# ATTron/astroz

Measured on AMD Instinct MI355X. Metric: propagations/sec, 13,478 sats x 1,440 times, at 1/2/4/8 MI355X, higher is better.
Workload: dtype f64

## Files before the change

astroz_amd/_native.py:

```python
import ctypes as C
import os

import numpy as np

_HERE = os.path.dirname(os.path.abspath(__file__))
LIB_PATH = os.environ.get("ASTROZ_AMD_LIB") or os.path.join(_HERE, "libastroz_hip.so")

WGS84, WGS72 = 0, 1
OUT_TEME, OUT_ECEF, OUT_GEODETIC, OUT_TOPOCENTRIC = 0, 1, 2, 3
SAT_MAJOR, TIME_MAJOR = 0, 1
OUTPUT_MODES = {"teme": OUT_TEME, "ecef": OUT_ECEF, "geodetic": OUT_GEODETIC, "topocentric": OUT_TOPOCENTRIC}
PASS_DTYPE = np.dtype([("t_rise_min", "<f8"), ("t_culm_min", "<f8"), ("t_set_min", "<f8"), ("max_elevation_rad", "<f8"),
                       ("rise_azimuth_rad", "<f8"), ("set_azimuth_rad", "<f8"), ("flags", "<u4"), ("grid_rise", "<u4"),
                       ("grid_culm", "<u4"), ("grid_set", "<u4")])
PASS_UP_AT_START, PASS_UP_AT_END, PASS_CUT_BY_ERROR = 1, 2, 4
ECLIPSE_DTYPE = np.dtype([("t_entry_min", "<f8"), ("t_exit_min", "<f8"), ("flags", "<u4"), ("grid_entry", "<u4"),
                          ("grid_exit", "<u4"), ("reserved", "<u4")])
ECLIPSE_IN_AT_START, ECLIPSE_IN_AT_END, ECLIPSE_CUT_BY_ERROR = 1, 2, 4
SHADOW_UMBRA, SHADOW_PENUMBRA = 0, 1
SHADOW_KINDS = {"umbra": SHADOW_UMBRA, "penumbra": SHADOW_PENUMBRA}
ACCESS_DTYPE = np.dtype([("t_start_min", "<f8"), ("t_end_min", "<f8"), ("min_range_km", "<f8"), ("flags", "<u4"),
                         ("grid_start", "<u4"), ("grid_end", "<u4"), ("grid_min_range", "<u4")])
ACCESS_OPEN_AT_START, ACCESS_OPEN_AT_END, ACCESS_CUT_BY_ERROR = 1, 2, 4
CONJUNCTION_DTYPE = np.dtype([("t_tca_min", "<f8"), ("miss_km", "<f8"), ("rel_speed_km_s", "<f8"), ("target", "<u4"),
                              ("sat", "<u4"), ("grid_index", "<u4"), ("reserved", "<u4")])

COVERAGE_DTYPE = np.dtype([("mean_in_view", "<f8"), ("max_gap_min", "<f8"), ("n_covered", "<u4"), ("min_in_view", "<u4"),
                           ("max_in_view", "<u4"), ("n_gaps", "<u4"), ("grid_gap_start", "<u4"), ("grid_gap_end", "<u4"),
                           ("flags", "<u4"), ("reserved", "<u4")])
COVERAGE_GAP_AT_START, COVERAGE_GAP_AT_END = 1, 2

AZ_ERR_HIP = -200
PATH_ROWS_FAST, PATH_TILES_FAST, PATH_ROWS_GENERIC, PATH_LANE_SAT, PATH_DEEP_ROWS, PATH_QUASI_UNIFORM, PATH_COLS_FAST, PATH_HOST_STEP = 1, 2, 4, 8, 16, 32, 64, 128

EXPORTS = [
    "astroz_version", "astroz_init", "astroz_deinit", "tle_parse", "tle_free",
    "tle_get_satellite_number", "tle_get_epoch", "tle_get_inclination", "tle_get_eccentricity",
    "tle_get_mean_motion", "sgp4_init", "sgp4_free", "sgp4_propagate", "sgp4_propagate_batch",
    "azh_device_count", "azh_last_error", "azh_parse_tle_lines", "azh_constellation_from_tle_text",
    "azh_constellation_from_tle_lines", "azh_constellation_from_elements", "azh_constellation_subset", "azh_constellation_free",
    "azh_num_satellites", "azh_num_sgp4", "azh_num_sdp4", "azh_get_epochs", "azh_get_status",
    "azh_get_field", "azh_propagate_host", "azh_propagate_device", "azh_propagate_device_cached", "azh_propagate_device_window",
    "azh_propagate_jd_host", "azh_synchronize", "azh_propagate_one_host", "azh_set_time_tile", "azh_set_timing", "azh_set_fast_path", "azh_set_tile_kernel", "azh_set_graphs", "azh_set_f32_arithmetic", "azh_set_f32_mode",
    "azh_last_kernel_ms", "azh_last_path", "azh_last_one_stats", "azh_set_host_copy_threads", "azh_set_host_points", "azh_get_host_points", "azh_selftest_coords", "azh_selftest_host_step", "azh_host_alloc", "azh_host_free", "azh_host_pool_stats", "azh_host_pool_trim", "azh_propagate_device_f32", "azh_propagate_device_cached_f32",
    "azh_screen_target_host", "azh_screen_target_device", "azh_coarse_screen_device", "azh_coarse_screen_host",
    "azh_screen_all_host", "azh_constellation_from_omm_json", "azh_propagate_one_device", "azh_selftest_math",
    "azh_parse_tle_text", "azh_parse_omm_json", "azh_set_parse_threads", "coords_julian_to_gmst",
    "azh_group_create_from_tle_text", "azh_group_create_from_omm_json", "azh_group_free", "azh_group_num_satellites",
    "azh_group_num_devices", "azh_group_padded_rows", "azh_group_get_epochs", "azh_group_propagate_host",
    "azh_group_propagate_allgather", "azh_group_screen_target_host", "azh_group_screen_target_device", "azh_group_shard_size",
    "azh_group_shard_rows", "azh_group_synchronize", "azh_screen_track_device", "coords_eci_to_ecef", "coords_ecef_to_geodetic",
    "orbital_hohmann", "orbital_velocity", "orbital_period", "orbital_escape_velocity",
    "azh_coords_topocentric", "azh_set_observer", "azh_find_passes_host", "azh_find_passes_device",
    "azh_find_passes_stations_host", "azh_find_passes_stations_device",
    "azh_coverage_host", "azh_coverage_device",
    "azh_sun_position_teme", "azh_selftest_sun", "azh_shadow_state", "azh_find_eclipses_host", "azh_find_eclipses_device",
    "azh_line_of_sight", "azh_find_access_host", "azh_find_access_device", "azh_find_access_track_device",
    "azh_closest_approach", "azh_find_conjunctions_host", "azh_find_conjunctions_device",
]


def _stations(stations, min_elevation_deg):
    st = np.ascontiguousarray(stations, dtype=np.float64).reshape(-1, 3)
    mk = np.ascontiguousarray(np.broadcast_to(np.asarray(min_elevation_deg, dtype=np.float64), (len(st),)))
    return st, mk


def _targets(targets):
    a = np.atleast_1d(np.asarray(targets))
    if a.ndim != 1 or a.size == 0 or a.dtype == np.bool_ or not np.issubdtype(a.dtype, np.integer) or (a < 0).any():
        raise ValueError("targets must be a satellite index or a non-empty sequence of them")
    return np.ascontiguousarray(a, dtype=np.uintp)


def _min_satellites(k):
    if isinstance(k, bool) or not isinstance(k, (int, np.integer)) or not 1 <= int(k) <= 0xFFFFFFFF:
        raise ValueError("min_satellites must be an integer >= 1")
    return int(k)


class NativeError(RuntimeError):
    def __init__(self, code, what):
        self.code = code
        super().__init__("%s failed with code %d%s" % (what, code, _detail(code)))


_lib = None


def _detail(code):
    if _lib is not None and code == AZ_ERR_HIP:
        msg = _lib.azh_last_error().decode(errors="replace")
        return " (%s)" % msg if msg else " (HIP runtime error: is an MI355X visible?)"
    return ""


def _share_hip_runtime_with_torch():
    if os.environ.get("ASTROZ_AMD_SYSTEM_HIP"):
        return
    import importlib.util
    try:
        spec = importlib.util.find_spec("torch")
    except (ImportError, ValueError):
        spec = None
    if spec is None or not spec.origin:
        return
    cand = os.path.join(os.path.dirname(spec.origin), "lib", "libamdhip64.so")
    if os.path.exists(cand):
        C.CDLL(cand, mode=C.RTLD_GLOBAL)


def lib():
    global _lib
    if _lib is not None:
        return _lib
    if not os.path.exists(LIB_PATH):
        raise ImportError(
            "astroz_amd: %s not found -- build it with `python -c 'import __graft_entry__ as g; "
            "g.build()'` (hipcc --offload-arch=gfx950). There is no CPU fallback." % LIB_PATH)
    _share_hip_runtime_with_torch()
    L = C.CDLL(LIB_PATH)
    vp, sz, dbl, i32, u32 = C.c_void_p, C.c_size_t, C.c_double, C.c_int32, C.c_uint32
    L.astroz_version.restype = u32
    L.tle_parse.argtypes = [C.c_char_p, C.POINTER(vp)]
    L.tle_parse.restype = i32
    L.tle_free.argtypes = [vp]
    L.tle_get_satellite_number.argtypes = [vp]
# ... 41 lines not shown
    L.azh_group_screen_target_device.restype = i32
    L.azh_group_shard_size.argtypes = [vp, i32]
    L.azh_group_shard_size.restype = sz
    L.azh_group_shard_rows.argtypes = [vp, i32, vp]
    L.azh_group_shard_rows.restype = i32
    L.azh_group_synchronize.argtypes = [vp]
    L.azh_group_synchronize.restype = i32
    L.azh_constellation_from_omm_json.argtypes = [C.c_char_p, sz, i32, i32, C.POINTER(vp)]
    L.azh_constellation_from_omm_json.restype = i32
    L.azh_propagate_one_device.argtypes = [vp, sz, vp, sz, vp, vp, vp, vp]
    L.azh_propagate_one_device.restype = i32
    L.azh_selftest_math.argtypes = [vp, sz, vp, i32]
    L.azh_selftest_math.restype = i32
    L.coords_julian_to_gmst.argtypes = [dbl]
    L.coords_julian_to_gmst.restype = dbl
    L.coords_eci_to_ecef.argtypes = [vp, dbl, vp]
    L.coords_eci_to_ecef.restype = None
    L.coords_ecef_to_geodetic.argtypes = [vp, vp]
    L.coords_ecef_to_geodetic.restype = None
    L.azh_constellation_from_tle_lines.argtypes = [vp, vp, sz, i32, i32, C.POINTER(vp)]
    L.azh_constellation_from_tle_lines.restype = i32
    L.azh_constellation_from_elements.argtypes = [sz] + [vp] * 8 + [i32, i32, C.POINTER(vp)]
    L.azh_constellation_from_elements.restype = i32
    L.azh_constellation_subset.argtypes = [vp, vp, sz, i32, C.POINTER(vp)]
    L.azh_constellation_subset.restype = i32
    L.azh_constellation_free.argtypes = [vp]
    for f in ("azh_num_satellites", "azh_num_sgp4", "azh_num_sdp4"):
        getattr(L, f).argtypes = [vp]
        getattr(L, f).restype = sz
    L.azh_get_epochs.argtypes = [vp, vp]
    L.azh_get_epochs.restype = i32
    L.azh_get_status.argtypes = [vp, vp, vp, vp]
    L.azh_get_status.restype = i32
    L.azh_get_field.argtypes = [vp, C.c_char_p, vp]
    L.azh_get_field.restype = i32
    L.azh_propagate_host.argtypes = [vp, vp, sz, vp, vp, vp, i32, dbl, vp, i32, sz, vp]
    L.azh_propagate_host.restype = i32
    L.azh_propagate_device.argtypes = [vp, vp, sz, vp, vp, vp, i32, dbl, vp, i32, sz, vp, vp]
    L.azh_propagate_device.restype = i32
    L.azh_propagate_device_cached.argtypes = [vp, vp, vp, i32, sz, vp, vp]
    L.azh_propagate_device_cached.restype = i32
    L.azh_propagate_device_window.argtypes = [vp, sz, sz, vp, vp, i32, sz, vp, vp]
    L.azh_propagate_device_window.restype = i32
    L.azh_propagate_jd_host.argtypes = [vp, vp, vp, sz, vp, vp, i32, i32, vp]
    L.azh_propagate_jd_host.restype = i32
    L.azh_synchronize.argtypes = [vp]
    L.azh_synchronize.restype = i32
    L.azh_propagate_one_host.argtypes = [vp, sz, vp, sz, vp, vp, vp]
    L.azh_propagate_one_host.restype = i32
    L.azh_set_time_tile.argtypes = [vp, u32, u32]
    L.azh_set_time_tile.restype = i32
    L.azh_set_timing.argtypes = [vp, i32]
    L.azh_set_timing.restype = i32
    L.azh_set_fast_path.argtypes = [vp, i32]
    L.azh_set_fast_path.restype = i32
    L.azh_set_tile_kernel.argtypes = [vp, i32]
    L.azh_set_tile_kernel.restype = i32
    L.azh_set_graphs.argtypes = [vp, i32]
    L.azh_set_graphs.restype = i32
    L.azh_set_f32_arithmetic.argtypes = [vp, i32]
    L.azh_set_f32_arithmetic.restype = i32
    L.azh_set_f32_mode.argtypes = [vp, i32]
    L.azh_set_f32_mode.restype = i32
    L.azh_last_kernel_ms.argtypes = [vp]
    L.azh_last_kernel_ms.restype = dbl
    L.azh_set_host_copy_threads.argtypes = [i32]
    L.azh_set_host_copy_threads.restype = None
    L.azh_set_host_points.argtypes = [sz]
    L.azh_set_host_points.restype = None
    L.azh_get_host_points.argtypes = []
    L.azh_get_host_points.restype = sz
    L.azh_host_alloc.argtypes = [C.c_size_t, C.POINTER(C.c_void_p)]
    L.azh_host_alloc.restype = i32
    L.azh_host_free.argtypes = [C.c_void_p]
    L.azh_host_free.restype = None
    L.azh_host_pool_stats.argtypes = [C.POINTER(C.c_size_t), C.POINTER(C.c_size_t)]
    L.azh_host_pool_stats.restype = None
    L.azh_host_pool_trim.argtypes = []
    L.azh_host_pool_trim.restype = None
    L.azh_last_path.argtypes = [vp]
    L.azh_last_path.restype = u32
    L.azh_last_one_stats.argtypes = [vp, vp, vp]
    L.azh_last_one_stats.restype = C.c_int32
    L.azh_propagate_device_f32.argtypes = L.azh_propagate_device.argtypes
    L.azh_propagate_device_f32.restype = i32
    L.azh_propagate_device_cached_f32.argtypes = L.azh_propagate_device_cached.argtypes
    L.azh_propagate_device_cached_f32.restype = i32
    L.azh_screen_target_host.argtypes = [vp, vp, sz, vp, sz, dbl, dbl, vp, vp]
    L.azh_screen_target_host.restype = i32
    L.azh_screen_target_device.argtypes = [vp, vp, sz, vp, sz, dbl, dbl, vp, vp, vp]
    L.azh_screen_target_device.restype = i32
    L.azh_screen_track_device.argtypes = [vp, vp, sz, vp, vp, sz, dbl, vp, vp, vp]
    L.azh_screen_track_device.restype = i32
    L.azh_coarse_screen_device.argtypes = [vp, sz, sz, i32, sz, dbl, vp, vp, vp, sz, C.POINTER(sz), vp]
    L.azh_coarse_screen_device.restype = i32
    L.azh_coarse_screen_host.argtypes = [vp, sz, sz, i32, sz, dbl, vp, vp, vp, sz, C.POINTER(sz), i32]
    L.azh_coarse_screen_host.restype = i32
    L.azh_screen_all_host.argtypes = [vp, vp, sz, vp, dbl, vp, vp, sz, C.POINTER(sz)]
    L.azh_screen_all_host.restype = i32
    L.azh_coords_topocentric.argtypes = [vp, vp, dbl, vp, vp, vp]
    L.azh_coords_topocentric.restype = None
    L.azh_set_observer.argtypes = [vp, dbl, dbl, dbl]
    L.azh_set_observer.restype = i32
    L.azh_find_passes_host.argtypes = [vp, vp, sz, vp, dbl, dbl, vp, sz, vp]
    L.azh_find_passes_host.restype = i32
    L.azh_find_passes_device.argtypes = [vp, vp, sz, vp, dbl, dbl, vp, sz, vp, vp]
    L.azh_find_passes_device.restype = i32
    L.azh_find_passes_stations_host.argtypes = [vp, vp, sz, vp, dbl, vp, vp, sz, vp, sz, vp]
    L.azh_find_passes_stations_host.restype = i32
    L.azh_find_passes_stations_device.argtypes = [vp, vp, sz, vp, dbl, vp, vp, sz, vp, sz, vp, vp]
    L.azh_find_passes_stations_device.restype = i32
    L.azh_coverage_host.argtypes = [vp, vp, sz, vp, dbl, vp, vp, sz, u32, vp, vp]
    L.azh_coverage_host.restype = i32
    L.azh_coverage_device.argtypes = [vp, vp, sz, vp, dbl, vp, vp, sz, u32, vp, vp, vp]
    L.azh_coverage_device.restype = i32
    L.azh_sun_position_teme.argtypes = [dbl, vp]
    L.azh_sun_position_teme.restype = None
    L.azh_selftest_sun.argtypes = [vp, sz, vp, i32]
    L.azh_selftest_sun.restype = i32
    L.azh_shadow_state.argtypes = [vp, vp, vp, vp]
    L.azh_shadow_state.restype = i32
    L.azh_find_eclipses_host.argtypes = [vp, vp, sz, vp, dbl, i32, vp, sz, vp, vp]
    L.azh_find_eclipses_host.restype = i32
    L.azh_find_eclipses_device.argtypes = [vp, vp, sz, vp, dbl, i32, vp, sz, vp, vp, vp]
    L.azh_find_eclipses_device.restype = i32
    L.azh_line_of_sight.argtypes = [vp, vp, dbl, vp, vp]
    L.azh_line_of_sight.restype = i32
    L.azh_find_access_host.argtypes = [vp, vp, sz, vp, sz, dbl, dbl, vp, sz, vp, vp]
    L.azh_find_access_host.restype = i32
    L.azh_find_access_device.argtypes = [vp, vp, sz, vp, sz, dbl, dbl, vp, sz, vp, vp, vp]
    L.azh_find_access_device.restype = i32
    L.azh_find_access_track_device.argtypes = [vp, vp, sz, vp, vp, vp, sz, dbl, dbl, vp, sz, vp, vp, vp]
    L.azh_find_access_track_device.restype = i32
    L.azh_closest_approach.argtypes = [vp, vp, vp, vp, dbl, vp, vp, vp]
    L.azh_closest_approach.restype = i32
    L.azh_find_conjunctions_host.argtypes = [vp, vp, sz, vp, vp, sz, dbl, vp, sz, vp]
    L.azh_find_conjunctions_host.restype = i32
    L.azh_find_conjunctions_device.argtypes = [vp, vp, sz, vp, vp, sz, dbl, vp, sz, vp, vp]
    L.azh_find_conjunctions_device.restype = i32
    L.orbital_hohmann.argtypes = [dbl, dbl, dbl, vp]
    L.orbital_hohmann.restype = i32
    for f, n in (("orbital_velocity", 3), ("orbital_period", 2), ("orbital_escape_velocity", 2)):
        getattr(L, f).argtypes = [dbl] * n
        getattr(L, f).restype = dbl
    _lib = L
    return L


def check(code, what):
    if code != 0:
        raise NativeError(code, what)


def _f64(a):
    return np.ascontiguousarray(a, dtype=np.float64)


def _ptr(a):
    return None if a is None else a.ctypes.data


class DeviceConstellation:

    def __init__(self, handle):
        self._h = handle
        L = lib()
# ... 276 lines not shown

    def find_conjunctions(self, times_min, targets, threshold_km, offsets_min=None, *, max_events=65536):
        times = _f64(times_min)
        off = None if offsets_min is None else _f64(offsets_min)
        if off is not None and len(off) < self.n:
            raise ValueError("epoch_offsets must have at least num_satellites elements")
        tg = _targets(targets)
        out = np.zeros(int(max_events), dtype=CONJUNCTION_DTYPE)
        cnt = np.zeros(1, dtype=np.uint32)
        check(lib().azh_find_conjunctions_host(self._h, times.ctypes.data, len(times), _ptr(off), tg.ctypes.data, len(tg),
                                               float(threshold_km), out.ctypes.data if max_events else None, int(max_events),
                                               cnt.ctypes.data), "azh_find_conjunctions_host")
        return out[:min(int(cnt[0]), int(max_events))], int(cnt[0])

    def find_conjunctions_device(self, times_min, targets, threshold_km, offsets_min, d_out, max_events, d_n_events, *, stream=None):
        times = _f64(times_min)
        off = None if offsets_min is None else _f64(offsets_min)
        tg = _targets(targets)
        check(lib().azh_find_conjunctions_device(self._h, times.ctypes.data, len(times), _ptr(off), tg.ctypes.data, len(tg),
                                                 float(threshold_km), d_out, int(max_events), d_n_events, stream),
              "azh_find_conjunctions_device")

    def screen_all(self, times_min, threshold=10.0, offsets_min=None, max_results=10_000_000):
        times = _f64(times_min)
        off = None if offsets_min is None else _f64(offsets_min)
        pairs = np.empty((max_results, 2), dtype=np.uint32)
        tt = np.empty(max_results, dtype=np.uint32)
        k = C.c_size_t(0)
        check(lib().azh_screen_all_host(self._h, times.ctypes.data, len(times), _ptr(off), float(threshold),
                                        pairs.ctypes.data, tt.ctypes.data, max_results, C.byref(k)),
              "azh_screen_all_host")
        return pairs[:k.value].copy(), tt[:k.value].copy()

    def propagate_one(self, sat_index, tsince_min):
        t = _f64(np.atleast_1d(tsince_min))
        n = len(t)
        pos = result_empty((n, 3))
        vel = result_empty((n, 3))
        err = result_empty((n,), np.uint8)
        check(lib().azh_propagate_one_host(self._h, sat_index, t.ctypes.data, n, pos.ctypes.data, vel.ctypes.data,
                                           err.ctypes.data), "azh_propagate_one_host")
        return err, pos, vel

    def propagate_one_device(self, sat_index, d_tsince, n, d_pos, d_vel=None, d_err=None, stream=None):
        check(lib().azh_propagate_one_device(self._h, sat_index, d_tsince, n, d_pos, d_vel, d_err, stream),
              "azh_propagate_one_device")

    F32_MODES = {"mixed": 0, "packed": 1, "fp64": 2}

    def set_f32_arithmetic(self, mode):
        if isinstance(mode, (bool, np.bool_)):
            check(lib().azh_set_f32_arithmetic(self._h, 1 if mode else 0), "azh_set_f32_arithmetic")
            return
        m = self.F32_MODES[mode] if isinstance(mode, str) else int(mode)
        check(lib().azh_set_f32_mode(self._h, m), "azh_set_f32_mode")

    def set_fast_path(self, enabled):
        check(lib().azh_set_fast_path(self._h, 1 if enabled else 0), "azh_set_fast_path")

    def set_tile_kernel(self, enabled):
        check(lib().azh_set_tile_kernel(self._h, int(enabled) if not isinstance(enabled, bool) else (1 if enabled else 0)), "azh_set_tile_kernel")

    def set_graphs(self, enabled):
        check(lib().azh_set_graphs(self._h, 1 if enabled else 0), "azh_set_graphs")

    def set_timing(self, enabled):
        check(lib().azh_set_timing(self._h, 1 if enabled else 0), "azh_set_timing")

    def synchronize(self):
        check(lib().azh_synchronize(self._h), "azh_synchronize")

    def last_kernel_ms(self):
        return lib().azh_last_kernel_ms(self._h)

    def last_path(self):
        return int(lib().azh_last_path(self._h))

    def last_one_stats(self):
        a, b = C.c_uint32(0), C.c_uint32(0)
        check(lib().azh_last_one_stats(self._h, C.byref(a), C.byref(b)), "azh_last_one_stats")
        return int(a.value), int(b.value)


class DeviceGroup:

    def __init__(self, text, devices, grav=WGS72, n_chunks=4):
        b = text.encode() if isinstance(text, str) else bytes(text)
        dv = (C.c_int32 * len(devices))(*devices)
        h = C.c_void_p()
        fn = lib().azh_group_create_from_omm_json if b.lstrip()[:1] in (b"{", b"[") else lib().azh_group_create_from_tle_text
        check(fn(b, len(b), grav, dv, len(devices), n_chunks, C.byref(h)), "azh_group_create")
        self._h = h
        self.n = lib().azh_group_num_satellites(h)
        self.n_devices = lib().azh_group_num_devices(h)
        self.padded_rows = lib().azh_group_padded_rows(h)
        self.epochs = np.empty(self.n)
        check(lib().azh_group_get_epochs(h, self.epochs.ctypes.data), "azh_group_get_epochs")

    def close(self):
        if getattr(self, "_h", None):
            lib().azh_group_free(self._h)
            self._h = None

    def __del__(self):
        try:
            self.close()
        except Exception:
            pass

    def _offsets(self, offsets_min):
        if offsets_min is None:
            return None
        off = _f64(offsets_min)
        if off.ndim != 1 or len(off) < self.n:
            raise ValueError("epoch_offsets must have at least num_satellites elements")
        return off

    def propagate_host(self, times_min, offsets_min=None, *, velocities=True, mode=OUT_TEME, reference_jd=0.0, errors=False):
        t = _f64(times_min)
        off = self._offsets(offsets_min)
        pos = result_empty((self.n, len(t), 3))
        vel = result_empty((self.n, len(t), 3)) if velocities else None
        big = self.n * len(t) >= PINNED_MIN_BYTES
        err = (result_empty((self.n, len(t)), np.uint8) if big else np.zeros((self.n, len(t)), dtype=np.uint8)) if errors else None
        check(lib().azh_group_propagate_host(self._h, t.ctypes.data, len(t), _ptr(off), 0 if off is None else len(off), pos.ctypes.data, _ptr(vel), mode,
                                             float(reference_jd), _ptr(err)), "azh_group_propagate_host")
        return pos, vel, err

    def screen_target(self, times_min, target, threshold_km, offsets_min=None, reference_jd=0.0):
        t = _f64(times_min)
        off = self._offsets(offsets_min)
        d = np.empty(self.n)
        ti = np.empty(self.n, dtype=np.uint32)
        check(lib().azh_group_screen_target_host(self._h, t.ctypes.data, len(t), _ptr(off), 0 if off is None else len(off), int(target),
                                                 float(threshold_km), float(reference_jd), d.ctypes.data, ti.ctypes.data),
              "azh_group_screen_target_host")
        return d, ti

    def screen_target_device(self, times_min, target, threshold_km, d_dist_ptrs, d_t_ptrs, offsets_min=None):
        t = _f64(times_min)
        off = self._offsets(offsets_min)
        dd = (C.c_void_p * self.n_devices)(*d_dist_ptrs)
        tt = (C.c_void_p * self.n_devices)(*d_t_ptrs)
        check(lib().azh_group_screen_target_device(self._h, t.ctypes.data, len(t), _ptr(off), 0 if off is None else len(off), int(target),
                                                   float(threshold_km), 0.0, dd, tt), "azh_group_screen_target_device")

    def shard_size(self, slot):
        return int(lib().azh_group_shard_size(self._h, int(slot)))

    def shard_rows(self, slot):
        out = np.empty(self.shard_size(slot), dtype=np.uint32)
        check(lib().azh_group_shard_rows(self._h, int(slot), out.ctypes.data), "azh_group_shard_rows")
        return out

    def synchronize(self):
        check(lib().azh_group_synchronize(self._h), "azh_group_synchronize")

    def propagate_allgather(self, times_min, offsets_min, d_pos_ptrs, d_vel_ptrs=None):
        t = _f64(times_min)
        off = self._offsets(offsets_min)
        pp = (C.c_void_p * self.n_devices)(*d_pos_ptrs)
        vv = (C.c_void_p * self.n_devices)(*d_vel_ptrs) if d_vel_ptrs is not None else None
        check(lib().azh_group_propagate_allgather(self._h, t.ctypes.data, len(t), _ptr(off), 0 if off is None else len(off), pp, vv),
              "azh_group_propagate_allgather")


# ... 220 lines not shown
```

astroz_amd/csrc/astroz_hip.hip:

```cpp
#include "../../include/astroz_hip.h"

#include <hip/hip_runtime.h>
#include <dlfcn.h>
#include <rccl/rccl.h>

#include <algorithm>
#include <atomic>
#include <cmath>
#include <condition_variable>
#include <deque>
#include <map>
#include <cstdio>
#include <cstdlib>
#include <cstring>
#include <mutex>
#include <new>
#include <memory>
#include <string>
#include <thread>
#include <type_traits>
#include <vector>

#include "kernels.h"
#include "passes_kernel.h"
// ... 91 lines not shown
        cap = 0;
        if (!hip_ok(hipHostMalloc(&p, want, hipHostMallocDefault), "hipHostMalloc")) return AZ_ERR_HIP;
        cap = want;
        return AZ_OK;
    }
};

template <class H, hipError_t (*Create)(H *, unsigned), hipError_t (*Destroy)(H)>
class HipHandle {
  public:
    HipHandle() = default;
    HipHandle(HipHandle &&o) noexcept { swap(o); }
    HipHandle &operator=(HipHandle &&o) noexcept { swap(o); return *this; }
    ~HipHandle() { reset(); }
    void swap(HipHandle &o) noexcept { std::swap(h_, o.h_); std::swap(own_, o.own_); }
    hipError_t create(unsigned flags)
    {
        reset();
        own_ = true;
        return Create(&h_, flags);
    }
    void borrow(H h)
    {
        reset();
        h_ = h;
        own_ = false;
    }
    void reset()
    {
        if (h_ && own_) (void)Destroy(h_);
        h_ = nullptr;
    }
    bool owned() const { return h_ && own_; }
    operator H() const { return h_; }

  private:
    H h_ = nullptr;
    bool own_ = false;
};
using Stream = HipHandle<hipStream_t, hipStreamCreateWithFlags, hipStreamDestroy>;
using Event = HipHandle<hipEvent_t, hipEventCreateWithFlags, hipEventDestroy>;

constexpr int kStageSlots = 3;
constexpr size_t kStageChunk = size_t(16) << 20;
struct HostStager {
    Event ev[kStageSlots];
    PinnedBuf slot[kStageSlots];
    int32_t ensure()
    {
        for (int k = 0; k < kStageSlots; ++k) {
            if (slot[k].ensure(kStageChunk) != AZ_OK) return AZ_ERR_HIP;
            if (!ev[k] && !hip_ok(ev[k].create(hipEventDisableTiming), "hipEventCreate")) return AZ_ERR_HIP;
        }
        return AZ_OK;
    }
};
}

struct azh_constellation {
    int device = 0;
    size_t n = 0, n_pad = 0;
    AzGrav g{};
    Stream s_main, s_deep, s_ecc;
    Event ev_fork, ev_join, ev_fork2, ev_join2, ev_t0, ev_t1;
    Event ev_one;
    Event ev_graph;
    DevBuf<double> d_el;
    DevBuf<unsigned> d_flags;
    std::vector<unsigned> h_flags;
    std::vector<double> h_epoch;
    std::vector<double> h_raw[AZ_NUM_RAW];
    DevBuf<unsigned> d_list;
    std::vector<unsigned> h_list;
    unsigned n_sgp4 = 0, n_sdp4 = 0, n_bad = 0;
    DevBuf<double> d_times, d_offsets, d_sin, d_cos, d_seeds;
    DevBuf<double> d_node_cache;
    struct FastPlan {
        bool valid = false, mixed32 = false;
        unsigned tile_c = 0, tile_e = 0, n_list = 0, n_seg = 0, parity = 0;
        DevBuf<double> win;
        DevBuf<unsigned char> flag;
        DevBuf<unsigned> redo;
    } plan[4];
    DevBuf<double> d_inc;
    DevBuf<double> d_fast_rec;
    double uniform_step = 0.0;
    DevBuf<float> d_delta;
    double delta_max = 0.0;
    std::vector<float> h_delta;
    DevBuf<double> d_delta64;
    std::vector<double> h_delta64;
    bool delta_wide = false;
    double grid_t0 = 0.0;
    unsigned last_path = 0;
    DevBuf<double> d_tgt, d_part_d2, d_out_d;
    DevBuf<unsigned> d_part_t, d_out_t;
    DevBuf<double> d_one_t, d_one_o;
    DevBuf<unsigned char> d_one_e;
    DevBuf<unsigned> d_one_items;
    unsigned one_segments = 0;
    PinnedBuf h_stage;
    std::vector<double> h_times, h_offsets;
    std::vector<uint8_t> h_mask;
    double staged_ref_jd = 0.0;
    hipStream_t staged_stream = nullptr;
    bool staged_valid = false;
    PinnedBuf h_small;
    HostStager stager;
    bool seeds_valid = false;
    unsigned seeds_tile = 0;
    bool seeds_rows = false;
    DevBuf<unsigned char> d_mask;
    DevBuf<double> d_host_pos, d_host_vel;
    DevBuf<unsigned char> d_host_err;
    bool have_offsets = false, have_mask = false;
    AzObserver obs{};
    DevBuf<AzObserver> d_obs;
    bool have_observer = false, obs_dirty = false;
    DevBuf<double> d_pass_pos, d_pass_vel;
    DevBuf<unsigned char> d_pass_err;
    DevBuf<azh_pass> d_pass_out;
    DevBuf<uint32_t> d_pass_n;
    std::vector<AzStation> h_stations;
    DevBuf<AzStation> d_stations;
    DevBuf<azh_coverage> d_cov_stats;
    DevBuf<uint32_t> d_cov_counts;
    DevBuf<AzSunPoint> d_sun;
    DevBuf<azh_eclipse> d_ecl_out;
    DevBuf<unsigned char> d_ecl_state;
    DevBuf<double> d_acc_track;
    DevBuf<azh_access> d_acc_out;
    DevBuf<unsigned char> d_acc_state;
    DevBuf<double> d_conj_track;
    std::vector<unsigned> h_conj_slots;
    DevBuf<unsigned> d_conj_slots;
    DevBuf<azh_conjunction> d_conj_out;
    unsigned cached_n_times = 0;
    int cached_mode = 0;
    unsigned off_cat = 0;
    unsigned off_deep_cat = 0;
    unsigned off_rowmap = 0;
    unsigned off_rowmap2 = 0;
    struct LaunchGraph {
        const void *pos, *vel, *err;
        int layout, f32;
        size_t stride, row_lo, row_hi;
        hipStream_t st;
        unsigned sig_before, sig_after;
        unsigned path;
        unsigned seen;
        unsigned fails;
        hipGraph_t graph;
        hipGraphExec_t exec;
    };
    std::vector<LaunchGraph> graphs;
    int graphs_on = 0;
    bool capturing = false;
    int cols_kernel = 0;
    DevBuf<double> d_deep_tmp;
    bool tile_kernel = true;
    unsigned off_circ = 0, n_circ = 0;
    bool timed = false;
    bool timing = true;
    unsigned tile_sgp4 = 0, tile_sdp4 = 0;
    int f32_mode = 0;
    bool fast_path = true;
    std::vector<double> h_el;
    std::vector<std::pair<size_t, std::vector<double>>> h_cols;
    size_t h_cols_next = 0;
    ~azh_constellation();
};

namespace {

constexpr size_t kHostMirrorPad = 64;
constexpr size_t kHostCols = 256;
constexpr size_t kHostColsBeforeTable = 8;
constexpr size_t kHostTableMax = size_t(64) << 20;
std::atomic<size_t> g_host_points{[] {
    const char *e = getenv("ASTROZ_AMD_HOST_POINTS");
    return e ? (size_t)strtoull(e, nullptr, 10) : size_t(128);
}()};
inline size_t host_points() { return azhost::cpu_ok() ? g_host_points.load(std::memory_order_relaxed) : 0; }

constexpr int32_t AZ_RC_EAGER = 0x7a5eca9;
int set_device(const azh_constellation *c) { return hip_ok(hipSetDevice(c->device), "hipSetDevice") ? AZ_OK : AZ_ERR_HIP; }

hipStream_t small_stream(int device)
{
    static std::mutex mu;
    static std::map<int, hipStream_t> streams;
    std::lock_guard<std::mutex> lk(mu);
    auto it = streams.find(device);
    if (it != streams.end()) return it->second;
    hipStream_t s = nullptr;
    if (!hip_ok(hipStreamCreateWithFlags(&s, hipStreamNonBlocking), "hipStreamCreate")) return nullptr;
    streams[device] = s;
    return s;
}

void drop_graphs(azh_constellation *c);

int32_t build(const std::vector<double> (&cols)[AZ_NUM_RAW], size_t n, int grav, int device, azh_constellation **out)
{
    if (!out) return AZ_ERR_NULL_POINTER;
    *out = nullptr;
    if (n == 0) return AZ_ERR_VALUE;
    if (n > 0x7fffffffu) return AZ_ERR_VALUE;
    int ndev = 0;
    HIP_TRY(hipGetDeviceCount(&ndev));
    if (device < 0 || device >= ndev) {
        g_last_error = "no such HIP device";
        return AZ_ERR_HIP;
    }
    std::unique_ptr<azh_constellation> c(new (std::nothrow) azh_constellation());
    if (!c) return AZ_ERR_ALLOC_FAILED;
    c->device = device;
    c->n = n;
    c->n_pad = (n + 63) / 64 * 64;
    c->g = make_grav(grav);
    if (set_device(c.get()) != AZ_OK) return AZ_ERR_HIP;
    if (n > 16) {
        if (!hip_ok(c->s_main.create(hipStreamNonBlocking), "hipStreamCreate") ||
            !hip_ok(c->s_deep.create(hipStreamNonBlocking), "hipStreamCreate") ||
            !hip_ok(c->s_ecc.create(hipStreamNonBlocking), "hipStreamCreate") ||
            !hip_ok(c->ev_graph.create(hipEventDisableTiming | hipEventDisableSystemFence), "hipEventCreate"))
            return AZ_ERR_HIP;
    } else {
        c->s_main.borrow(small_stream(device));
        if (!c->s_main) return AZ_ERR_HIP;
        c->s_deep.borrow(c->s_main);
        c->s_ecc.borrow(c->s_main);
    }
    for (Event *e : {&c->ev_fork2, &c->ev_join2, &c->ev_fork, &c->ev_join, &c->ev_one})
        if (!hip_ok(e->create(hipEventDisableTiming), "hipEventCreate")) return AZ_ERR_HIP;
    if (!hip_ok(c->ev_t0.create(hipEventDefault), "hipEventCreate") || !hip_ok(c->ev_t1.create(hipEventDefault), "hipEventCreate"))
// ... 340 lines not shown
        with_vel_frame(vel, a.mode, [&](auto VEL, auto FRAME) { launch_rows_fast<VEL, FRAME, AZ_SINK_F64, true>(e, e.n_list, se); });
        if (se != st)
            if (int32_t rc = stream_after(st, se, side.join); rc != AZ_OK) return rc;
    }
    a.tile = shape.tile_c;
    a.ecc_row0 = ecc_row0;
    PropArgs r = a;
    r.tm_rows = 1;
    const dim3 grid(pad8((a.n_rows + 63u) / 64u), cgrid_y(a.n_times, a.tile));
    with_vel_frame(vel, a.mode, [&](auto VEL, auto FRAME) {
        with_bool(a.delta64 != nullptr, [&](auto WIDE) {
            hipLaunchKernelGGL((k_cols_fast<VEL, FRAME, WIDE ? 2 : 0>), grid, dim3(64), 0, st, a);
        });
        launch_redo<VEL, FRAME, AZ_SINK_F64>(r, dim3(256, 4), st);
    });
    return AZ_OK;
}

unsigned launch_propagate(const PropArgs &a, int layout, bool vel, bool deep, hipStream_t st)
{
    if (use_rows(a, layout, deep)) {
        PropArgs b = a;
        b.tile = rows_tile(a.n_list, a.n_times, a.tile_forced);
        if (deep) b.tile = std::min(b.tile, 64u * (unsigned)AZ_DEEP_SEED_MAX);
        const unsigned n_slots = a.slot_hi ? a.slot_hi - a.slot_lo : a.n_list;
        const dim3 grid(pad8(n_slots), cgrid_y(a.n_times, b.tile));
        with_outputs(a, vel, [&](auto VEL, auto FRAME, auto SINK) {
            if (deep) hipLaunchKernelGGL((k_rows_deep<VEL, gen_frame(FRAME), SINK>), grid, dim3(64), 0, st, b);
            else hipLaunchKernelGGL((k_rows<VEL, gen_frame(FRAME), SINK>), grid, dim3(64), 0, st, b);
        });
        return deep ? AZH_PATH_DEEP_ROWS : AZH_PATH_ROWS_GENERIC;
    }
    const dim3 grid(pad8((a.n_list + AZ_BLOCK - 1) / AZ_BLOCK), cgrid_y(a.n_times, a.tile));
    with_bool(deep, [&](auto DEEP) {
        if (a.screen_target)
            hipLaunchKernelGGL((k_propagate<0, false, DEEP, 0, true>), grid, dim3(AZ_BLOCK), 0, st, a);
        else
            with_bool(layout == AZ_LAYOUT_TIME_MAJOR, [&](auto TIME_MAJOR) {
                with_vel_frame(vel, a.mode, [&](auto VEL, auto FRAME) {
                    hipLaunchKernelGGL((k_propagate<TIME_MAJOR, VEL, DEEP, gen_frame(FRAME)>), grid, dim3(AZ_BLOCK), 0, st, a);
                });
            });
    });
    return AZH_PATH_LANE_SAT;
}

int32_t stage_inputs(azh_constellation *c, const double *times, size_t n_times, const double *offsets,
                     const uint8_t *mask, int mode, double reference_jd, hipStream_t st)
{
    if (n_times > 0xffffffffu) return AZ_ERR_VALUE;
    {
        const bool same = c->staged_valid && st == c->staged_stream && n_times == c->h_times.size() && mode == c->cached_mode &&
                          (mode == AZ_OUT_TEME || reference_jd == c->staged_ref_jd) &&
                          (offsets != nullptr) == c->have_offsets && (mask != nullptr) == c->have_mask &&
                          (n_times == 0 || memcmp(times, c->h_times.data(), sizeof(double) * n_times) == 0) &&
                          (!offsets || (c->h_offsets.size() == c->n && memcmp(offsets, c->h_offsets.data(), sizeof(double) * c->n) == 0)) &&
                          (!mask || (c->h_mask.size() == c->n && memcmp(mask, c->h_mask.data(), c->n) == 0));
        if (same) return AZ_OK;
        c->staged_valid = false;
    }
    if (c->d_times.ensure(n_times) != AZ_OK) return AZ_ERR_HIP;
    HIP_TRY(hipMemcpyAsync(c->d_times.p, times, sizeof(double) * n_times, hipMemcpyHostToDevice, st));
    c->have_offsets = offsets != nullptr;
    if (offsets) {
        if (c->d_offsets.ensure(c->n) != AZ_OK) return AZ_ERR_HIP;
        HIP_TRY(hipMemcpyAsync(c->d_offsets.p, offsets, sizeof(double) * c->n, hipMemcpyHostToDevice, st));
    }
    c->have_mask = mask != nullptr;
    if (mask) {
        if (c->d_mask.ensure(c->n) != AZ_OK) return AZ_ERR_HIP;
        HIP_TRY(hipMemcpyAsync(c->d_mask.p, mask, c->n, hipMemcpyHostToDevice, st));
    }
    if (mode != AZ_OUT_TEME) {
        if (c->d_sin.ensure(n_times) != AZ_OK || c->d_cos.ensure(n_times) != AZ_OK) return AZ_ERR_HIP;
        hipLaunchKernelGGL(k_gmst, dim3((unsigned)((n_times + 255) / 256)), dim3(256), 0, st, c->d_times.p,
                           (unsigned)n_times, reference_jd, c->d_sin.p, c->d_cos.p);
        HIP_TRY(hipGetLastError());
    }
    c->cached_n_times = (unsigned)n_times;
    c->cached_mode = mode;
    c->seeds_valid = false;
    drop_graphs(c);
    for (auto &pl : c->plan) pl.valid = false;
    c->uniform_step = 0.0;
    c->delta_max = 0.0;
    c->delta_wide = false;
    c->grid_t0 = n_times ? times[0] : 0.0;
    if (n_times >= 2) {
        double t0 = times[0], step = (times[n_times - 1] - t0) / (double)(n_times - 1);
        double tmax = std::max(std::fabs(t0), std::fabs(times[n_times - 1]));
        const double tol = 4.0 * 2.220446049250313e-16 * std::max(tmax, std::fabs(step));
        bool uni = std::isfinite(step) && step != 0.0;
        double dmax = 0.0;
        for (size_t i = 1; uni && i < n_times; ++i) {
            dmax = std::max(dmax, std::fabs(times[i] - std::fma((double)i, step, t0)));
            uni = dmax <= AZ_DELTA_MAX;
        }
        if (uni && dmax > tol) {
            c->h_delta.assign(n_times + AZ_DELTA_SEG, 0.0f);
            for (size_t i = 0; i < n_times; ++i) c->h_delta[i] = (float)(times[i] - std::fma((double)i, step, t0));
            if (c->d_delta.ensure(c->h_delta.size()) != AZ_OK) return AZ_ERR_HIP;
            HIP_TRY(hipMemcpyAsync(c->d_delta.p, c->h_delta.data(), sizeof(float) * c->h_delta.size(), hipMemcpyHostToDevice, st));
            c->h_delta64.assign(n_times + AZ_DELTA_SEG, 0.0);
            for (size_t i = 0; i < n_times; ++i) c->h_delta64[i] = times[i] - std::fma((double)i, step, t0);
            if (c->d_delta64.ensure(c->h_delta64.size()) != AZ_OK) return AZ_ERR_HIP;
            HIP_TRY(hipMemcpyAsync(c->d_delta64.p, c->h_delta64.data(), sizeof(double) * c->h_delta64.size(), hipMemcpyHostToDevice, st));
            c->delta_max = dmax * (1.0 + 1e-6) + 1e-12;
        }
        if (!uni && n_times >= 64) {
            const double nn = (double)n_times, im = 0.5 * (nn - 1.0);
            double tm = 0.0;
            for (size_t i = 0; i < n_times; ++i) tm += times[i];
            tm /= nn;
            double sxy = 0.0, sxx = 0.0;
            for (size_t i = 0; i < n_times; ++i) {
                sxy += ((double)i - im) * (times[i] - tm);
                sxx += ((double)i - im) * ((double)i - im);
            }
            step = sxy / sxx;
            t0 = tm - step * im;
            bool ok = std::isfinite(step) && std::isfinite(t0) && step != 0.0;
            dmax = 0.0;
            for (size_t i = 0; ok && i < n_times; ++i) {
                dmax = std::max(dmax, std::fabs(times[i] - std::fma((double)i, step, t0)));
                ok = dmax <= AZ_DELTA_WIDE_MAX;
            }
            if (ok && dmax <= 0.5 * std::fabs(step)) {
                c->h_delta64.assign(n_times + AZ_DELTA_SEG, 0.0);
                for (size_t i = 0; i < n_times; ++i) c->h_delta64[i] = times[i] - std::fma((double)i, step, t0);
                if (c->d_delta64.ensure(c->h_delta64.size()) != AZ_OK) return AZ_ERR_HIP;
                HIP_TRY(hipMemcpyAsync(c->d_delta64.p, c->h_delta64.data(), sizeof(double) * c->h_delta64.size(), hipMemcpyHostToDevice, st));
                c->delta_max = dmax * (1.0 + 1e-6) + 1e-12;
                c->delta_wide = true;
                c->grid_t0 = t0;
                uni = true;
            }
        }
        if (uni) {
            if (c->d_inc.ensure((size_t)2 * AZ_INC_NUM * c->n_pad) != AZ_OK) return AZ_ERR_HIP;
            hipLaunchKernelGGL(k_prep_inc, dim3((unsigned)((c->n + 255) / 256)), dim3(256), 0, st, c->d_el.p, c->n, c->n_pad,
                               step, c->d_inc.p);
            HIP_TRY(hipGetLastError());
            if (c->d_fast_rec.ensure((size_t)FR_NUM * c->n_pad) != AZ_OK) return AZ_ERR_HIP;
            hipLaunchKernelGGL(k_prep_rec, dim3((unsigned)((c->n + 255) / 256)), dim3(256), 0, st, c->d_el.p, c->d_flags.p, c->n, c->n_pad,
                               c->d_inc.p, c->d_fast_rec.p);
            HIP_TRY(hipGetLastError());
            c->uniform_step = step;
        }
    }
    try {
        c->h_times.assign(times, times + n_times);
        if (offsets) c->h_offsets.assign(offsets, offsets + c->n);
        if (mask) c->h_mask.assign(mask, mask + c->n);
        c->staged_ref_jd = reference_jd;
        c->staged_stream = st;
        c->staged_valid = true;
    } catch (const std::bad_alloc &) {
        c->staged_valid = false;
    }
    return AZ_OK;
}

int32_t prepare_deep(azh_constellation *c, PropArgs &d, hipStream_t st, bool rows, bool beside_bulk = false)
{
    const unsigned n_times = d.n_times;
    d.list = c->d_list.p + (rows ? c->off_deep_cat : c->n_sgp4);
    d.n_list = c->n_sdp4;
    d.tile = auto_tile(c->n_sdp4, n_times, c->tile_sdp4, 8);
    d.tile_forced = c->tile_sdp4 ? c->tile_sdp4 : (rows && beside_bulk && c->n_sgp4 >= 4u * c->n_sdp4 ? rows_tile(c->n_sgp4, n_times, c->tile_sgp4) : 0u);
    const unsigned seed_tile = rows ? 64u : d.tile;
    const unsigned n_tiles = (n_times + seed_tile - 1) / seed_tile;
    if (!c->seeds_valid || c->seeds_tile != seed_tile || c->seeds_rows != rows) {
        if (c->capturing) return AZ_RC_EAGER;
        drop_graphs(c);
        if (c->d_seeds.ensure((size_t)n_tiles * 3 * c->n_sdp4) != AZ_OK) return AZ_ERR_HIP;
        if (c->d_node_cache.p == nullptr) {
            if (c->d_node_cache.ensure(3 * c->n_pad) != AZ_OK) return AZ_ERR_HIP;
            HIP_TRY(hipMemsetAsync(c->d_node_cache.p, 0, sizeof(double) * 3 * c->n_pad, st));
        }
        hipLaunchKernelGGL(k_deep_seed, dim3((c->n_sdp4 + 63) / 64), dim3(64), 0, st, c->d_el.p, c->d_flags.p, c->n_pad,
                           d.list, c->n_sdp4, d.times, n_times, d.offsets, seed_tile, c->d_seeds.p, rows ? 1 : 0, c->d_node_cache.p);
        HIP_TRY(hipGetLastError());
        c->seeds_valid = true;
        c->seeds_tile = seed_tile;
        c->seeds_rows = rows;
    }
    d.seeds = c->d_seeds.p;
    return AZ_OK;
}

int32_t ensure_plan(azh_constellation *c, PropArgs &a, const FastShape &shape, hipStream_t st)
{
    azh_constellation::FastPlan &pl = c->plan[shape.kind];
    const unsigned n_list = a.n_list;
    const unsigned n_seg = (a.n_times + std::min(shape.tile_c, shape.tile_e) - 1) / std::min(shape.tile_c, shape.tile_e);
    if (!pl.valid || pl.tile_c != shape.tile_c || pl.tile_e != shape.tile_e || pl.n_list != n_list || pl.mixed32 != shape.mixed32) {
        if (c->capturing) return AZ_RC_EAGER;
        drop_graphs(c);
        const size_t items = (size_t)n_list * n_seg + ((size_t)a.n_times + 63) / 64 * (c->n_sgp4 - c->n_circ);
        if (pl.redo.cap < 4 + 3 * items || pl.win.cap < (size_t)n_list * n_seg * AZ_PLAN_NUM) HIP_TRY(hipStreamSynchronize(st));
        if (pl.redo.ensure(4 + 3 * items) != AZ_OK || pl.win.ensure((size_t)n_list * n_seg * AZ_PLAN_NUM) != AZ_OK ||
            pl.flag.ensure((size_t)n_list * n_seg) != AZ_OK)
            return AZ_ERR_HIP;
        HIP_TRY(hipMemsetAsync(pl.redo.p, 0, 4 * sizeof(unsigned), st));
        PlanArgs q{};
        q.el = a.el; q.flags = a.flags; q.n_pad = a.n_pad; q.list = a.list; q.n_list = n_list; q.n_circ = a.n_circ;
        q.n_times = a.n_times; q.tile_c = shape.tile_c; q.tile_e = shape.tile_e; q.by_flags = shape.kind == 2 ? 1u : 0u;
        q.times = a.times; q.offsets = a.offsets; q.inc = a.inc; q.step = a.uniform_step; q.dt_mult = shape.kind == 1 ? 128.0 : 64.0;
        q.delta_max = (a.delta || a.delta64) ? a.delta_max : 0.0;
        q.grid_t0 = a.grid_t0;
        q.f32_mixed = shape.mixed32 ? 1u : 0u;
        q.win = pl.win.p; q.flag = pl.flag.p;
        q.redo_static = pl.redo.p + 2; q.redo_c0 = pl.redo.p; q.redo_c1 = pl.redo.p + 1; q.redo_items = pl.redo.p + 4;
        q.g = a.g;
        hipLaunchKernelGGL(k_plan_windows, dim3((n_list + 255) / 256, n_seg), dim3(256), 0, st, q);
        hipLaunchKernelGGL(k_plan_arm, dim3(1), dim3(64), 0, st, q.redo_static, q.redo_c0, q.redo_c1);
        HIP_TRY(hipGetLastError());
        pl.valid = true;
        pl.tile_c = shape.tile_c; pl.tile_e = shape.tile_e; pl.n_list = n_list; pl.n_seg = n_seg; pl.parity = 0; pl.mixed32 = shape.mixed32;
    }
    a.plan_win = pl.win.p;
    a.plan_flag = pl.flag.p;
    a.plan_stride = n_list;
    a.redo_static = pl.redo.p + 2;
    a.redo_count = pl.redo.p + pl.parity;
    a.redo_next = pl.redo.p + (pl.parity ^ 1u);
    a.redo_items = pl.redo.p + 4;
    pl.parity ^= 1u;
    return AZ_OK;
}

void drop_graphs(azh_constellation *c)
{
    if (c->graphs.empty()) return;
    if (hipEventSynchronize(c->ev_graph) != hipSuccess) (void)hipGetLastError();
    for (auto &g : c->graphs) {
        if (g.exec) (void)hipGraphExecDestroy(g.exec);
        if (g.graph) (void)hipGraphDestroy(g.graph);
    }
    c->graphs.clear();
}
}

azh_constellation::~azh_constellation()
{
    (void)hipSetDevice(device);
    drop_graphs(this);
}

namespace {
unsigned plan_sig(const azh_constellation *c)
{
    unsigned s = 0;
    for (unsigned k = 0; k < 4; ++k) s |= (c->plan[k].parity & 1u) << k;
    return s;
}

int32_t launch_all(azh_constellation *c, double *d_pos, double *d_vel, int layout, size_t stride, uint8_t *d_err,
                   hipStream_t st, int f32 = 0, size_t row_lo = 0, size_t row_hi = ~(size_t)0)
{
    const unsigned n_times = c->cached_n_times;
    if (n_times == 0) return AZ_OK;
    row_hi = std::min(row_hi, c->n);
    if (row_lo >= row_hi) return AZ_OK;
    if (stride == 0) stride = c->n;
    if (layout == AZ_LAYOUT_TIME_MAJOR && stride < c->n) return AZ_ERR_VALUE;

    PropArgs a{};
    a.el = c->d_el.p;
    a.flags = c->d_flags.p;
    a.n_pad = c->n_pad;
    a.times = c->d_times.p;
    a.n_times = n_times;
    a.offsets = c->have_offsets ? c->d_offsets.p : nullptr;
    a.pos = d_pos;
    a.vel = d_vel;
    a.sin_g = c->d_sin.p;
    a.cos_g = c->d_cos.p;
    a.mask = c->have_mask ? c->d_mask.p : nullptr;
    a.err = d_err;
    a.stride_sats = stride;
    a.mode = c->cached_mode;
    if (a.mode == AZ_OUT_TOPOCENTRIC) {
        if (c->obs_dirty) {
            if (c->capturing) return AZ_RC_EAGER;
            if (c->d_obs.ensure(1) != AZ_OK) return AZ_ERR_HIP;
            HIP_TRY(hipMemcpyAsync(c->d_obs.p, &c->obs, sizeof(AzObserver), hipMemcpyHostToDevice, st));
            c->obs_dirty = false;
        }
        a.obs = c->d_obs.p;
    }
    a.f32 = f32;
    a.arith32 = f32 ? c->f32_mode : 2;
    a.g = c->g;
    a.uniform_step = c->fast_path ? c->uniform_step : 0.0;
    a.inc = (a.uniform_step != 0.0) ? c->d_inc.p : nullptr;
    a.fast_rec = (a.uniform_step != 0.0) ? c->d_fast_rec.p : nullptr;
    a.delta = (a.uniform_step != 0.0 && c->delta_max > 0.0 && !c->delta_wide) ? c->d_delta.p : nullptr;
    a.delta64 = (a.uniform_step != 0.0 && c->delta_max > 0.0) ? c->d_delta64.p : nullptr;
    a.delta_wide = c->delta_wide ? 1 : 0;
    a.grid_t0 = c->grid_t0;
    a.delta_max = c->delta_max;
    a.grid_exact_uniform = (c->uniform_step != 0.0 && c->delta_max == 0.0) ? 1 : 0;
    a.row_lo = (unsigned)row_lo;
    a.row_hi = (unsigned)row_hi;
    const bool windowed = row_lo > 0 || row_hi < c->n;
    auto slots_of = [&](unsigned off, unsigned cnt, unsigned &lo, unsigned &hi) {
        const unsigned *b = c->h_list.data() + off, *e = b + cnt;
        lo = (unsigned)(std::lower_bound(b, e, (unsigned)row_lo) - b);
        hi = (unsigned)(std::lower_bound(b, e, (unsigned)row_hi) - b);
    };
    unsigned deep_lo = 0, deep_hi = 0;
    if (windowed) {
        slots_of(c->off_circ, c->n_circ, a.win_circ_lo, a.win_circ_hi);
        slots_of(c->off_circ + c->n_circ, c->n_sgp4 - c->n_circ, a.win_ecc_lo, a.win_ecc_hi);
        slots_of(c->off_deep_cat, c->n_sdp4, deep_lo, deep_hi);
    }

    unsigned path = 0;
    if (c->timing) HIP_TRY(hipEventRecord(c->ev_t0, st));
    if (d_err) HIP_TRY(hipMemsetAsync(d_err + row_lo * (size_t)n_times, 0, (row_hi - row_lo) * (size_t)n_times, st));
    const bool tiles = c->n_sgp4 > 0 && c->tile_kernel && a.inc != nullptr && layout == AZ_LAYOUT_TIME_MAJOR && !f32 &&
                       n_times >= 64 &&
                       (size_t)stride * 64 * 24 < 0xf0000000ull;
    const bool cols = tiles && c->cols_kernel != 0 && a.mask == nullptr;
    const unsigned n_ecc = c->n_sgp4 - c->n_circ;
    const size_t scratch_rows = (size_t)c->n_sdp4 + (cols ? n_ecc : 0u);
    const size_t scratch_per = scratch_rows * n_times * 3, scratch_words = f32 ? (scratch_per + 1) / 2 : scratch_per;
    auto ensure_scratch = [&](hipStream_t user) -> int32_t {
        if (c->capturing && c->d_deep_tmp.cap < scratch_words * (d_vel ? 2 : 1)) return AZ_RC_EAGER;
        if (c->d_deep_tmp.cap < scratch_words * (d_vel ? 2 : 1)) {
            drop_graphs(c);
            HIP_TRY(hipStreamSynchronize(user));
        }
        if (c->d_deep_tmp.ensure(scratch_words * (d_vel ? 2 : 1)) != AZ_OK) return AZ_ERR_HIP;
        a.tmp_pos = c->d_deep_tmp.p;
        a.tmp_vel = d_vel ? c->d_deep_tmp.p + scratch_words : nullptr;
        return AZ_OK;
    };
    const bool fork = c->n_sdp4 > 0;
    if (cols && !fork && n_ecc)
        if (int32_t rc = ensure_scratch(st); rc != AZ_OK) return rc;
    if (fork) {
        if (int32_t rc = stream_after(c->s_deep, st, c->ev_fork); rc != AZ_OK) return rc;
        PropArgs d = a;
        const bool deep_rows = use_rows(d, layout, true);
        const bool deep_skip = windowed && deep_rows && deep_hi == deep_lo;
        if (windowed && deep_rows) { d.slot_lo = deep_lo; d.slot_hi = deep_hi; }
        if (int32_t rc = prepare_deep(c, d, c->s_deep, deep_rows, !tiles && a.inc != nullptr); rc != AZ_OK) return rc;
// ... 8 lines not shown
            dim3 tg((c->n_sdp4 + AZ_TR_ROWS - 1) / AZ_TR_ROWS, (n_times + 63) / 64);
            if (tiles || deep_skip) {  }
            else if (f32)
                hipLaunchKernelGGL((k_deep_transpose<float>), tg, dim3(192), 0, c->s_deep, reinterpret_cast<const float *>(t.pos),
                                   reinterpret_cast<const float *>(t.vel), reinterpret_cast<float *>(d_pos), reinterpret_cast<float *>(d_vel),
                                   d.list, c->n_sdp4, n_times, stride, d.mask, d.row_lo, d.row_hi);
            else
                hipLaunchKernelGGL((k_deep_transpose<double>), tg, dim3(192), 0, c->s_deep, t.pos, t.vel, d_pos, d_vel, d.list, c->n_sdp4,
                                   n_times, stride, d.mask, d.row_lo, d.row_hi);
        } else if (!deep_skip) {
            path |= launch_propagate(d, layout, d_vel != nullptr, true, c->s_deep);
        }
        HIP_TRY(hipGetLastError());
        HIP_TRY(hipEventRecord(c->ev_join, c->s_deep));
    }
    if (c->n_sgp4 > 0) {
        a.list = c->d_list.p;
        a.n_list = c->n_sgp4;
        a.tile = auto_tile(c->n_sgp4, n_times, c->tile_sgp4, 8);
        a.tile_forced = c->tile_sgp4;
        if (tiles && fork) HIP_TRY(hipStreamWaitEvent(st, c->ev_join, 0));
        if (tiles && !cols) a.list = c->d_list.p + c->off_cat;
        FastShape shape;
        const bool fast = a.inc != nullptr && (tiles || use_rows(a, layout, false));
        if (fast) {
            if (!tiles || cols) a.list = c->d_list.p + c->off_circ;
            a.n_list = c->n_sgp4;
            a.n_circ = c->n_circ;
            a.rowmap = c->d_list.p + (cols ? c->off_rowmap2 : c->off_rowmap);
            a.n_rows = (unsigned)c->n;
            shape = cols ? fast_shape_cols(a, (unsigned)c->n, c->n_sgp4, c->n_circ)
                         : (tiles ? fast_shape_tiles(a, (unsigned)c->n) : fast_shape_rows(a, c->n_sgp4, c->n_circ));
            if (int32_t rc = ensure_plan(c, a, shape, st); rc != AZ_OK) return rc;
        }
        const EccSide side{c->s_ecc, c->ev_fork2, c->ev_join2};
        if (a.n_list > 0 && cols) {
            if (int32_t rc = launch_cols(a, d_vel != nullptr, st, shape, side, c->n_sdp4); rc != AZ_OK) return rc;
            path |= AZH_PATH_COLS_FAST;
        } else if (a.n_list > 0 && tiles) {
            launch_tiles(a, d_vel != nullptr, st, shape);
            path |= AZH_PATH_TILES_FAST;
        } else if (a.n_list > 0 && fast) {
            const dim3 rgrid(std::min(8192u, std::max(256u, (a.n_list * cgrid_y(a.n_times, shape.tile_c) + 63u) / 64u)), 4);
            if (int32_t rc = launch_near_fast(a, d_vel != nullptr, shape, rgrid, st, side); rc != AZ_OK) return rc;
            path |= AZH_PATH_ROWS_FAST;
        } else if (a.n_list > 0) {
            path |= launch_propagate(a, layout, d_vel != nullptr, false, st);
        }
        if ((a.delta || a.delta64) && (path & (AZH_PATH_TILES_FAST | AZH_PATH_ROWS_FAST | AZH_PATH_COLS_FAST))) path |= AZH_PATH_QUASI_UNIFORM;
        HIP_TRY(hipGetLastError());
    }
    if (c->n_bad > 0) {
        hipLaunchKernelGGL(k_fill_bad, dim3((n_times + 255) / 256, c->n_bad), dim3(256), 0, st,
                           c->d_list.p + c->n_sgp4 + c->n_sdp4, c->n_bad, c->d_flags.p, n_times, d_pos, d_vel, d_err,
                           c->have_mask ? c->d_mask.p : nullptr, layout, stride, f32, a.row_lo, a.row_hi);
        HIP_TRY(hipGetLastError());
    }
    if (fork && !tiles) HIP_TRY(hipStreamWaitEvent(st, c->ev_join, 0));
    c->last_path = path;
    if (c->timing) {
        HIP_TRY(hipEventRecord(c->ev_t1, st));
        c->timed = true;
    }
    return AZ_OK;
}

int32_t launch_cached(azh_constellation *c, double *d_pos, double *d_vel, int layout, size_t stride, uint8_t *d_err, hipStream_t st,
                      int f32 = 0, size_t row_lo = 0, size_t row_hi = ~(size_t)0)
{
    if (!c->graphs_on || c->timing || c->cached_n_times == 0 || !c->s_main.owned()) return launch_all(c, d_pos, d_vel, layout, stride, d_err, st, f32, row_lo, row_hi);
    const unsigned sig = plan_sig(c);
    azh_constellation::LaunchGraph *hit = nullptr, *pending = nullptr;
    for (auto &g : c->graphs)
        if (g.pos == d_pos && g.vel == d_vel && g.err == d_err && g.layout == layout && g.f32 == f32 && g.stride == stride &&
            g.row_lo == row_lo && g.row_hi == row_hi && g.st == st) {
            if (g.fails >= 2) return launch_all(c, d_pos, d_vel, layout, stride, d_err, st, f32, row_lo, row_hi);
            if (g.exec && g.sig_before == sig) { hit = &g; break; }
            if (!g.exec && g.sig_before == sig) pending = &g;
        }
    if (hit) {
        HIP_TRY(hipGraphLaunch(hit->exec, st));
        for (unsigned k = 0; k < 4; ++k) c->plan[k].parity = (hit->sig_after >> k) & 1u;
        c->last_path = hit->path;
        HIP_TRY(hipEventRecord(c->ev_graph, st));
        return AZ_OK;
    }
    if (!pending) {
        if (c->graphs.size() >= 24) drop_graphs(c);
        const int32_t rc = launch_all(c, d_pos, d_vel, layout, stride, d_err, st, f32, row_lo, row_hi);
        if (rc == AZ_OK) {
            try {
                c->graphs.push_back({d_pos, d_vel, d_err, layout, f32, stride, row_lo, row_hi, st, sig, plan_sig(c), c->last_path, 1u, 0u, nullptr, nullptr});
            } catch (const std::bad_alloc &) {
            }
        }
        return rc;
    }
    if (hipStreamBeginCapture(st, hipStreamCaptureModeThreadLocal) != hipSuccess) {
        (void)hipGetLastError();
        return launch_all(c, d_pos, d_vel, layout, stride, d_err, st, f32, row_lo, row_hi);
    }
    unsigned parity0[4];
    for (unsigned k = 0; k < 4; ++k) parity0[k] = c->plan[k].parity;
    c->capturing = true;
    const int32_t rc = launch_all(c, d_pos, d_vel, layout, stride, d_err, st, f32, row_lo, row_hi);
    c->capturing = false;
    hipGraph_t graph = nullptr;
    const hipError_t e_end = hipStreamEndCapture(st, &graph);
    hipGraphExec_t exec = nullptr;
    if (rc != AZ_OK || e_end != hipSuccess || !graph || hipGraphInstantiate(&exec, graph, nullptr, nullptr, 0) != hipSuccess) {
        (void)hipGetLastError();
        if (graph) (void)hipGraphDestroy(graph);
        for (unsigned k = 0; k < 4; ++k) c->plan[k].parity = parity0[k];
        pending->fails += 1;
        if (rc != AZ_OK && rc != AZ_RC_EAGER) return rc;
        return launch_all(c, d_pos, d_vel, layout, stride, d_err, st, f32, row_lo, row_hi);
    }
    pending->graph = graph;
    pending->exec = exec;
    pending->sig_after = plan_sig(c);
    pending->path = c->last_path;
    HIP_TRY(hipGraphLaunch(exec, st));
    HIP_TRY(hipEventRecord(c->ev_graph, st));
    return AZ_OK;
}

class HostPool {
  public:
    int32_t alloc(size_t bytes, void **out)
    {
        if (!out) return AZ_ERR_NULL_POINTER;
        *out = nullptr;
        const size_t need = std::max<size_t>((bytes + kGrain - 1) / kGrain * kGrain, kGrain);
        {
            std::lock_guard<std::mutex> lock(mu_);
            auto it = free_.lower_bound(need);
            if (it != free_.end() && it->first <= need + need / 4 + kGrain) {
                void *q = it->second;
                free_bytes_ -= it->first;
                live_[static_cast<char *>(q)] = it->first;
                free_.erase(it);
                *out = q;
                return AZ_OK;
            }
        }
        void *q = nullptr;
        if (hipHostMalloc(&q, need, hipHostMallocPortable) != hipSuccess || !q) {
            (void)hipGetLastError();
            trim(0);
            if (!hip_ok(hipHostMalloc(&q, need, hipHostMallocPortable), "hipHostMalloc(result)")) return AZ_ERR_ALLOC_FAILED;
        }
        std::lock_guard<std::mutex> lock(mu_);
        live_[static_cast<char *>(q)] = need;
        *out = q;
        return AZ_OK;
    }
    void release(void *q)
    {
        if (!q) return;
        {
            std::lock_guard<std::mutex> lock(mu_);
            auto it = live_.find(static_cast<char *>(q));
            if (it == live_.end()) return;
            free_.emplace(it->second, q);
            free_bytes_ += it->second;
            live_.erase(it);
        }
        trim(cap());
    }
    bool owns(const void *q, size_t len)
    {
        if (!q) return false;
        std::lock_guard<std::mutex> lock(mu_);
        auto it = live_.upper_bound(const_cast<char *>(static_cast<const char *>(q)));
        if (it == live_.begin()) return false;
        --it;
        return static_cast<const char *>(q) + len <= it->first + it->second;
    }
    void stats(size_t *live_bytes, size_t *free_bytes)
    {
        std::lock_guard<std::mutex> lock(mu_);
        size_t l = 0;
        for (auto &kv : live_) l += kv.second;
        if (live_bytes) *live_bytes = l;
        if (free_bytes) *free_bytes = free_bytes_;
    }
    void trim(size_t keep)
    {
        std::vector<void *> drop;
        {
            std::lock_guard<std::mutex> lock(mu_);
            while (free_bytes_ > keep && !free_.empty()) {
                auto it = std::prev(free_.end());
                drop.push_back(it->second);
                free_bytes_ -= it->first;
                free_.erase(it);
            }
        }
        for (void *q : drop) (void)hipHostFree(q);
    }

  private:
    static constexpr size_t kGrain = size_t(2) << 20;
    static size_t cap()
// ... 1745 lines not shown
            if (rc != AZ_OK) {
                (void)hipStreamSynchronize(c->s_main);
                return rc;
            }
            const char *h = static_cast<const char *>(c->h_small.p);
            memcpy(pos, h, bytes);
            if (vel) memcpy(vel, h + o_vel, bytes);
            if (err) memcpy(err, h + o_err, err_bytes);
            return AZ_OK;
        }
        if (c->d_host_pos.ensure(words) != AZ_OK || (vel && c->d_host_vel.ensure(words) != AZ_OK) ||
            (err && c->d_host_err.ensure(c->n * n_times) != AZ_OK))
            return AZ_ERR_HIP;
        double *d_pos = c->d_host_pos.p, *d_vel = vel ? c->d_host_vel.p : nullptr;
        uint8_t *d_err = err ? c->d_host_err.p : nullptr;
        int32_t rc = AZ_OK;
        do {
            const bool partial = mask != nullptr || (layout == AZ_LAYOUT_TIME_MAJOR && stride > c->n);
            if (partial) {
                if (!hip_ok(hipMemcpyAsync(d_pos, pos, bytes, hipMemcpyHostToDevice, c->s_main), "H2D pos")) { rc = AZ_ERR_HIP; break; }
                if (vel && !hip_ok(hipMemcpyAsync(d_vel, vel, bytes, hipMemcpyHostToDevice, c->s_main), "H2D vel")) { rc = AZ_ERR_HIP; break; }
            }
            rc = azh_propagate_device(c, times, n_times, offsets, d_pos, d_vel, mode, reference_jd, mask, layout, stride, d_err, nullptr);
            if (rc != AZ_OK) break;
            void *const dst[3] = {pos, vel, err};
            const void *const src[3] = {d_pos, d_vel, d_err};
            const size_t len[3] = {bytes, vel ? bytes : 0, err ? c->n * n_times : 0};
            const unsigned thr = host_copy_threads();
            const bool pinned_out = host_pool().owns(pos, bytes) && (!vel || host_pool().owns(vel, bytes));
            if (!pinned_out && thr > 0 && len[0] + len[1] + len[2] >= (size_t(8) << 20)) {
                if ((rc = copy_back_staged(c->stager, dst, src, len, 3, c->s_main, thr)) != AZ_OK) break;
            } else {
                for (int k = 0; k < 3 && rc == AZ_OK; ++k)
                    if (len[k] && !hip_ok(hipMemcpyAsync(dst[k], src[k], len[k], hipMemcpyDeviceToHost, c->s_main), "D2H")) rc = AZ_ERR_HIP;
                if (rc != AZ_OK) break;
            }
            if (!hip_ok(hipStreamSynchronize(c->s_main), "sync")) { rc = AZ_ERR_HIP; break; }
        } while (0);
        if (rc != AZ_OK) (void)hipStreamSynchronize(c->s_main);
        return rc;
    });
}

int32_t azh_propagate_jd_host(azh_constellation *c, const double *jd, const double *fr, size_t n_times, double *pos,
                              double *vel, int32_t mode, int32_t layout, uint8_t *err)
{
    return guarded([&]() -> int32_t {
        if (!c || !jd || !fr || !pos) return AZ_ERR_NULL_POINTER;
        double ref = c->h_epoch.empty() ? 0.0 : c->h_epoch[0];
        for (size_t s = 0; s < c->n; ++s)
            if (AZ_FLAG_ERR(c->h_flags[s]) == 0 && !(c->h_flags[s] & AZ_FLAG_DEEP)) { ref = c->h_epoch[s]; break; }
        std::vector<double> times(n_times), offs(c->n);
        for (size_t t = 0; t < n_times; ++t) times[t] = ((jd[t] + fr[t]) - ref) * 1440.0;
        for (size_t s = 0; s < c->n; ++s) offs[s] = (ref - c->h_epoch[s]) * 1440.0;
        return azh_propagate_host(c, times.data(), n_times, offs.data(), pos, vel, mode, ref, nullptr, layout, 0, err);
    });
}

int32_t azh_synchronize(azh_constellation *c)
{
    if (!c) return AZ_ERR_NULL_POINTER;
    if (set_device(c) != AZ_OK) return AZ_ERR_HIP;
    HIP_TRY(hipStreamSynchronize(c->s_deep));
    HIP_TRY(hipStreamSynchronize(c->s_ecc));
    HIP_TRY(hipStreamSynchronize(c->s_main));
    return AZ_OK;
}

uint32_t azh_last_path(const azh_constellation *c) { return c ? c->last_path : 0u; }

int32_t azh_last_one_stats(azh_constellation *c, uint32_t *n_segments, uint32_t *n_handed_over)
{
    if (!c || !n_segments || !n_handed_over) return AZ_ERR_NULL_POINTER;
    *n_segments = c->one_segments;
    *n_handed_over = 0;
    if (c->one_segments == 0) return AZ_OK;
    if (set_device(c) != AZ_OK) return AZ_ERR_HIP;
    HIP_TRY(hipEventSynchronize(c->ev_one));
    unsigned head[AZ_ONE_HEAD];
    HIP_TRY(hipMemcpy(head, c->d_one_items.p, sizeof(head), hipMemcpyDeviceToHost));
    unsigned cnt = 0;
    for (unsigned k = 0; k < AZ_ONE_LISTS; ++k) cnt += head[32u * k];
    *n_handed_over = cnt;
    return AZ_OK;
}

double azh_last_kernel_ms(azh_constellation *c)
{
    if (!c || !c->timed) return -1.0;
    float ms = -1.0f;
    if (hipEventElapsedTime(&ms, c->ev_t0, c->ev_t1) != hipSuccess) {
        (void)hipGetLastError();
        return -1.0;
    }
    return (double)ms;
}

int32_t azh_propagate_one_host(azh_constellation *c, size_t sat, const double *tsince, size_t n, double *pos,
                               double *vel, uint8_t *err)
{
    return guarded([&]() -> int32_t {
        if (!c || !tsince || !pos) return AZ_ERR_NULL_POINTER;
        if (sat >= c->n) return AZ_ERR_VALUE;
        if (n == 0) return AZ_OK;
        return run_one_satellite(c, sat, tsince, n, 0, nullptr, pos, vel, err);
    });
}

int32_t azh_propagate_one_device(azh_constellation *c, size_t sat, const double *d_tsince, size_t n, double *d_pos,
                                 double *d_vel, uint8_t *d_err, void *stream)
{
    return guarded([&]() -> int32_t {
        if (!c || !d_tsince || !d_pos) return AZ_ERR_NULL_POINTER;
        if (sat >= c->n || n > 0xffffffffu) return AZ_ERR_VALUE;
        if (n == 0) return AZ_OK;
        if (set_device(c) != AZ_OK) return AZ_ERR_HIP;
        hipStream_t st = stream ? (hipStream_t)stream : c->s_main;
        if (c->timing) HIP_TRY(hipEventRecord(c->ev_t0, st));
        if (int32_t lrc = launch_one(c, sat, d_tsince, n, d_pos, d_vel, d_err, 0, st); lrc != AZ_OK) return lrc;
        if (c->timing) {
            HIP_TRY(hipEventRecord(c->ev_t1, st));
            c->timed = true;
        }
        return AZ_OK;
    });
}

int32_t azh_selftest_math(const double *x, size_t n, double *out6n, int32_t device)
{
    if (!x || !out6n) return AZ_ERR_NULL_POINTER;
    if (n == 0) return AZ_OK;
    HIP_TRY(hipSetDevice(device));
    DevBuf<double> d;
    if (d.ensure(7 * n) != AZ_OK) return AZ_ERR_HIP;
    if (!hip_ok(hipMemcpy(d.p, x, sizeof(double) * n, hipMemcpyHostToDevice), "H2D")) return AZ_ERR_HIP;
    hipLaunchKernelGGL(k_math_kat, dim3((unsigned)((n + 63) / 64)), dim3(64), 0, nullptr, d.p, (unsigned)n, d.p + n);
    if (!hip_ok(hipGetLastError(), "k_math_kat") ||
        !hip_ok(hipMemcpy(out6n, d.p + n, sizeof(double) * 6 * n, hipMemcpyDeviceToHost), "D2H"))
        return AZ_ERR_HIP;
    return AZ_OK;
}

int32_t azh_selftest_host_step(const double *el, size_t n_pad, size_t sat, uint32_t flags, int32_t grav, const double *tsince_min,
                               size_t n, double *out6n, uint8_t *err)
{
    if (!el || !tsince_min || !out6n) return AZ_ERR_NULL_POINTER;
    if (sat >= n_pad) return AZ_ERR_VALUE;
    if (!azhost::cpu_ok()) return AZ_ERR_UNKNOWN;
    azhost::propagate_points(el, n_pad, sat, flags, make_grav(grav), tsince_min, n, 1, out6n, nullptr, nullptr, err);
    return AZ_OK;
}

struct azh_group {
    int n_dev = 0;
    size_t n = 0, rows = 0, n_chunks = 1;
    std::vector<int> devices;
    std::vector<std::unique_ptr<azh_constellation>> shard;
    std::vector<std::vector<uint32_t>> members;
    std::vector<std::vector<double>> off_stage;
    std::vector<double> track_stage;
    std::vector<ncclComm_t> comms;
    std::vector<Stream> s_comm;
    std::vector<Event> ev;
    size_t cell_lo(size_t chunk, int d) const { return std::min((chunk * n_dev + d) * rows, n); }
    size_t cell_hi(size_t chunk, int d) const { return std::min((chunk * n_dev + d) * rows + rows, n); }
    size_t padded() const { return n_chunks * n_dev * rows; }
// ... 623 lines not shown
```

astroz_amd/csrc/fast_step.h:

```cpp
#pragma once
#include <type_traits>

#include "propagate_device.h"

#define AZ_FASTK_COLD(X)                                                                                     \
    X(cc1) X(d2) X(d3) X(d4) X(nl2) X(nl3) X(nl4) X(nl5) X(eta) X(omgcof) X(xmcof) X(xd) X(bc4) X(bc5) X(ecb) X(sab)
#define AZ_FASTK_HOT(X)                                                                                      \
    X(aycof) X(xlcof) X(xnodcf) X(sinio) X(cosio) X(k_mrt) X(k_c2u) X(k_su) X(k_node) X(k_inc) X(x1mth2) X(k_rv) \
    X(sdA) X(cdA) X(sdW) X(cdW) X(tc) X(sdU) X(cdU) X(tmid) X(nodedot) X(sOc) X(cOc)
enum FastCold {
#define X(n) FC_##n,
    AZ_FASTK_COLD(X)
#undef X
    FC_NUM
};
#define AZ_FASTK_DELTA(X) X(mdot) X(argpdot) X(udot)
enum FastColdX {
    FCX_first_ = FC_NUM - 1,
#define X(n) FCX_##n,
    AZ_FASTK_DELTA(X)
#undef X
    FCX_NUM
};
#define AZ_DELTA_MAX 4.0e-6
// ... 217 lines not shown

#define AZ_ROT_16TH 0.0625
template <class RC>
AZ_DEVICE void az_pq_16th(double d, const RC &k, double &p, double &q)
{
    const double d2 = d * d;
    q = d2 * fma(d2, fma(d2, fma(d2, k(RC_p40320), k(RC_n720)), k(RC_p24)), -0.5);
    p = d * fma(d2, fma(d2, fma(d2, k(RC_n5040), k(RC_p120)), k(RC_n6)), 1.0);
}

template <class RC>
AZ_DEVICE void az_pq_large(double d, const RC &k, double &p, double &q)
{
    const double d2 = d * d;
    q = fma(d2, k(RC_p16f), k(RC_n14f));
    q = fma(d2, q, k(RC_p12f));
    q = fma(d2, q, k(RC_n3628800));
    q = fma(d2, q, k(RC_p40320));
    q = fma(d2, q, k(RC_n720));
    q = fma(d2, q, k(RC_p24));
    q = d2 * fma(d2, q, -0.5);
    p = fma(d2, k(RC_n15f), k(RC_p13f));
    p = fma(d2, p, k(RC_n11f));
    p = fma(d2, p, k(RC_p362880));
    p = fma(d2, p, k(RC_n5040));
    p = fma(d2, p, k(RC_p120));
    p = fma(d2, p, k(RC_n6));
    p = d * fma(d2, p, 1.0);
}

template <class RC>
AZ_DEVICE void az_pq_med(double d, const RC &k, double &p, double &q)
{
    const double d2 = d * d;
    q = fma(d2, k(RC_n3628800), k(RC_p40320));
    q = fma(d2, q, k(RC_n720));
    q = fma(d2, q, k(RC_p24));
    q = d2 * fma(d2, q, -0.5);
    p = fma(d2, k(RC_p362880), k(RC_n5040));
    p = fma(d2, p, k(RC_p120));
    p = fma(d2, p, k(RC_n6));
    p = d * fma(d2, p, 1.0);
}


template <bool SCALAR>
AZ_DEVICE void az_pair_advance(double &s, double &c, double sd, double cd)
{
#ifndef AZ_HOST_EMUL
    if (SCALAR) {
        double m, m2;
        asm("v_mul_f64 %2, %1, %4\n\t"
            "v_mul_f64 %3, %0, %4\n\t"
            "v_fma_f64 %0, %0, %5, %2\n\t"
            "v_fma_f64 %1, %1, %5, -%3"
            : "+v"(s), "+v"(c), "=&v"(m), "=&v"(m2)
            : "s"(sd), "s"(cd));
        return;
    }
#endif
    const double ns = fma(s, cd, c * sd);
    c = fma(c, cd, -(s * sd));
    s = ns;
}

template <class RC>
AZ_DEVICE void az_pq_ecc_scaled(double d, const RC &k, double &p, double &q)
{
    const double d2 = d * d;
    q = d2 * fma(d2, k(RC_p24), -0.5);
    p = d * fma(d2, fma(d2, k(RC_p120), k(RC_n6)), 1.0);
}
template <class RC>
AZ_DEVICE void az_fpq_milli(double d, const RC &k, double &p, double &q)
{
    const double d2 = d * d;
    q = d2 * fma(d2, k(RC_p24), -0.5);
    p = fma(d2 * k(RC_n6), d, d);
}

#define AZ_FAST_EL2 1.6e-5
#define AZ_FAST_TEMP2 6.0e-4

template <bool ECC>
AZ_DEVICE bool az_fast_window_ok(const FastK &k, const AzGrav &g, double t_a, double t_b, double dmax = 0.0)
{
    const double T = fmax(fabs(t_a), fabs(t_b)) + dmax;
    const double ae = fabs(k.eta_);
    const double th = fma(fabs(k.xmcof_), ae * fma(2.0 * ae, ae, 6.0), fabs(k.omgcof_) * T);
    const double da = T * fma(T, fma(T, fma(T, fabs(k.d4_), fabs(k.d3_)), fabs(k.d2_)), fabs(k.cc1_));
    const double em = fabs(k.ecb_) + fma(fabs(k.bc4_), T, fabs(k.bc5_));
    bool ok = (th <= AZ_ROT_16TH) & (da <= 0.25) & (em <= 0.9);
    const double sam = k.sab_ * (1.0 - da);
    const double inv_am = 1.0 / (sam * sam);
    const double temp = inv_am / fma(-em, em, 1.0);
    const double el = fma(temp, fabs(k.aycof_), em);
    const double el2 = el * el;
    if (!ECC) ok &= el2 <= AZ_FAST_EL2;
    ok &= el2 <= 0.81;
    const double dc = fmax(fabs(t_a - k.tc_), fabs(t_b - k.tc_)) + dmax;
    const double eps = fma(temp * fabs(k.xlcof_), em, fma(fabs(k.nl2_) * dc, dc, T * T * T * fma(T, fma(T, fabs(k.nl5_), fabs(k.nl4_)), fabs(k.nl3_)))) +
                       fabs(k.udot_) * dmax;
    ok &= eps <= AZ_ROT_MED;
    const double inv_pl = inv_am / (1.0 - el2);
    const double temp2 = g.half_j2 * inv_pl * inv_pl;
    ok &= temp2 <= AZ_FAST_TEMP2;
    const double a_nd = fma(fabs(k.k_node_), temp2, fma(fabs(k.nodedot_), 0.5 * fabs(t_b - t_a) + dmax, fabs(k.xnodcf_) * T * T));
    ok &= a_nd <= AZ_ROT_MED;
    return ok;
}

template <bool VEL, bool ECC = false, int DELTA = 0, class K = FastK, class RC = RotCoefLit>
AZ_DEVICE bool az_sgp4_fast_step(const K &k, const AzGrav &g, const RC &rk, double t, FastCarry &st, double r[3],
                                  double v[3], double dl = 0.0)
{
    az_pair_advance<K::SCALAR>(st.sA, st.cA, k.sdA(), k.cdA());
    az_pair_advance<K::SCALAR>(st.sW, st.cW, k.sdW(), k.cdW());
    az_pair_advance<K::SCALAR>(st.sU, st.cU, k.sdU(), k.cdU());
    double sA = st.sA, cA = st.cA, sW = st.sW, cW = st.cW;
    if constexpr ((DELTA == 1 && ECC) || DELTA == 2) {
        const double a = k.mdot() * dl, b = k.argpdot() * dl;
        if constexpr (DELTA == 2 && ECC) {
            double pa, qa;
            az_pq_16th(a, rk, pa, qa);
            az_rot_apply2(sA, cA, pa, qa);
        } else if constexpr (DELTA == 2) {
            az_rotate_tiny2(sA, cA, a, rk);
        } else {
            sA = fma(st.cA, a, st.sA); cA = fma(-st.sA, a, st.cA);
        }
        if constexpr (DELTA == 2 && ECC) az_rotate_tiny2(sW, cW, b, rk);
        else { sW = fma(st.cW, b, st.sW); cW = fma(-st.sW, b, st.cW); }
    }
    const double t2 = t * t;

    const double dm = fma(k.eta(), cA, 1.0);
    const double th = fma(k.xmcof(), dm * dm * dm, fma(k.omgcof(), t, -k.xd()));
    const double tempa = fma(-t, fma(t, fma(t, fma(t, k.d4(), k.d3()), k.d2()), k.cc1()), 1.0);
    const double dtc = t - k.tc();
    double nl = fma(k.nl2() * dtc, dtc, t2 * (t * fma(t, fma(t, k.nl5(), k.nl4()), k.nl3())));
    if constexpr (DELTA != 0) nl = fma(k.udot(), dl, nl);
    bool bad = false;
    double p, q;
    if (ECC) az_pq_16th(th, rk, p, q);
    else az_pq_ecc_scaled(th, rk, p, q);
    const double smm = fma(cA, p, fma(sA, q, sA));
    const double sw = fma(-cW, p, fma(sW, q, sW));
    const double cw = fma(sW, p, fma(cW, q, cW));
    const double em = fmax(fma(-k.bc5(), smm, fma(-k.bc4(), t, k.ecb())), 1.0e-6);

    const double sqrt_am = k.sab() * fabs(tempa);
    const double am = sqrt_am * sqrt_am;
    const double omem2 = fma(-em, em, 1.0);
    const double R = az_rcp(sqrt_am * omem2);
    const double ra = R * omem2;
    const double temp = ra * R;

    const double axnl = em * cw;
    const double aynl = fma(em, sw, temp * k.aycof());
    double s = st.sU, c = st.cU;
    {
        const double eps = fma(temp * k.xlcof(), axnl, nl);
        az_pq_16th(eps, rk, p, q);
        az_rot_apply2(s, c, p, q);
    }

    const double el2 = fma(axnl, axnl, aynl * aynl);
    double ecose, esine, ome, inv_ome, betal, inv_omel2, inv_1pb;
    if (!ECC) {
        const double rden = az_rcp1(fma(-s, aynl, fma(-c, axnl, 1.0)));
        const double d0 = fma(axnl, s, -(aynl * c)) * rden;
        az_fpq_milli(d0, rk, p, q);
        az_rot_apply2(s, c, p, q);
        const double d1 = fma(axnl, s, fma(-aynl, c, -d0)) * rden;
        {
            const double s1 = fma(c, d1, s);
            c = fma(-s, d1, c);
            s = s1;
        }
        ecose = fma(axnl, c, aynl * s);
        esine = fma(axnl, s, -(aynl * c));
        ome = 1.0 - ecose;
        const double x = fma(-ome, rden, 1.0);
        inv_ome = fma(rden, fma(x, x, x), rden);
        betal = fma(el2, fma(el2, -0.125, -0.5), 1.0);
        inv_omel2 = el2 + 1.0;
        inv_1pb = fma(el2, rk(RC_p8), 0.5);
    } else {
        double eps = 0.0, rden = 1.0, d = 0.0;
#pragma unroll
        for (int it = 0; it < 5; ++it) {
            rden = az_rcp1(fma(-s, aynl, fma(-c, axnl, 1.0)));
            d = fma(axnl, s, fma(-aynl, c, -eps)) * rden;
            eps += d;
            if (it == 0) {
                bad |= !(fabs(d) <= 0.5);
                az_pq_large(d, rk, p, q);
                az_rot_apply2(s, c, p, q);
            } else if (it == 1) {
                bad |= !(fabs(d) <= AZ_ROT_MED);
                az_pq_med(d, rk, p, q);
                az_rot_apply2(s, c, p, q);
            } else {
                bad |= !(fabs(d) <= AZ_ROT_SMALL);
                az_fpq_small(d, rk, p, q);
                az_rot_apply2(s, c, p, q);
            }
        }
        const double d2 = d * d;
        bad |= !(el2 * d2 * d2 < 4.0e-26);
        ecose = fma(axnl, c, aynl * s);
        esine = fma(axnl, s, -(aynl * c));
        ome = 1.0 - ecose;
        inv_ome = fma(rden, fma(-ome, rden, 1.0), rden);
        const double omel2 = 1.0 - el2;
        const double rb = az_rsqrt(omel2);
        betal = omel2 * rb;
        inv_omel2 = rb * rb;
        inv_1pb = az_rcp(1.0 + betal);
    }

    const double est = esine * inv_1pb;
    const double sinu = inv_ome * (s - fma(axnl, est, aynl));
    const double cosu = inv_ome * (c + fma(aynl, est, -axnl));
    const double sin2u = (sinu + sinu) * cosu;
    const double cos2u = fma(-2.0 * sinu, sinu, 1.0);

    const double inv_am = ra * ra;
    const double rl = am * ome;
    const double inv_pl = inv_am * inv_omel2;
    const double temp1 = g.half_j2 * inv_pl;
    const double temp2 = temp1 * inv_pl;

    const double mrt = fma(rl, fma(k.k_mrt() * temp2, betal, 1.0), k.k_c2u() * temp1 * cos2u);
    const double t2s = temp2 * sin2u;
    const double a_nd = fma(k.k_node(), t2s, fma(k.nodedot(), t - k.tmid(), k.xnodcf() * t2));
    double ssu = sinu, csu = cosu, sn = k.sOc(), cn = k.cOc(), si = k.sinio(), ci = k.cosio();
    az_rotate_tiny2(ssu, csu, k.k_su() * t2s, rk);
    az_pq_16th(a_nd, rk, p, q);
    az_rot_apply2(sn, cn, p, q);
    az_rotate_tiny2(si, ci, k.k_inc() * temp2 * cos2u, rk);

    const double xmx = -sn * ci, xmy = cn * ci;
    const double ux = fma(xmx, ssu, cn * csu);
    const double uy = fma(xmy, ssu, sn * csu);
    const double uz = si * ssu;
    const double rs = mrt * g.radius_km;
    r[0] = rs * ux;
    r[1] = rs * uy;
    r[2] = rs * uz;
    if (VEL) {
        const double rv = ra * g.vkmpersec;
        const double vk = rv * inv_ome;
        const double nxt = rv * inv_am * temp1;
        const double mvt = fma(-nxt * k.x1mth2(), sin2u, vk * esine);
        const double rvdot = fma(nxt, fma(k.x1mth2(), cos2u, k.k_rv()), vk * betal);
        const double vx = fma(xmx, csu, -(cn * ssu));
        const double vy = fma(xmy, csu, -(sn * ssu));
        const double vz = si * csu;
        v[0] = fma(mvt, ux, rvdot * vx);
        v[1] = fma(mvt, uy, rvdot * vy);
        v[2] = fma(mvt, uz, rvdot * vz);
    }
    return bad;
}
```

astroz_amd/csrc/kernels.h:

```cpp
#pragma once
#include <hip/hip_runtime.h>

#include <type_traits>

#include "init_device.h"
#include "propagate_device.h"
#include "fast_step.h"
#include "fast_step_f32.h"

#ifndef AZ_BLOCK
#define AZ_BLOCK 256
#endif
#ifndef AZ_PROP_FAST
#define AZ_PROP_FAST 1
#endif
#ifndef AZ_MIN_WAVES
#define AZ_MIN_WAVES 1
#endif
#ifndef AZ_ROWS_WAVES
#define AZ_ROWS_WAVES 3
#endif
#ifndef AZ_DEEP_WAVES
#define AZ_DEEP_WAVES 2
#endif
#define AZ_RESEED 256
#ifndef AZ_SM_CHUNK
#define AZ_SM_CHUNK 4
#endif

struct PropArgs {
    const double *el;
    const unsigned *flags;
    size_t n_pad;
    const unsigned *list;
    unsigned n_list;
    const double *times;
    unsigned n_times;
    const double *offsets;
    double *pos, *vel;
    const double *sin_g, *cos_g;
    const unsigned char *mask;
    unsigned char *err;
    size_t stride_sats;
    unsigned tile;
    unsigned tile_e, screen_nseg;
    unsigned tile_forced;
    const double *seeds;
    int mode;
    int f32;
    int tm_rows;
    int rows_compact;
    unsigned ecc_row0;
    const double *screen_target;
    union {
        double *part_d2;
        const AzObserver *obs;
    };
    unsigned *part_t;
    double uniform_step;
    int grid_exact_uniform;
    const float *delta;
    double delta_max;
    const double *delta64;
    int delta_wide;
    double grid_t0;
    const double *inc;
    const double *fast_rec;
    unsigned row_lo, row_hi;
    unsigned slot_lo, slot_hi;
    unsigned win_circ_lo, win_circ_hi, win_ecc_lo, win_ecc_hi;
    int arith32;
    unsigned n_circ;
    unsigned redo_slot0;
    unsigned *redo_count;
    unsigned *redo_next;
    unsigned *redo_items;
    const unsigned *rowmap;
    const double *tmp_pos, *tmp_vel;
    unsigned n_rows;
    const double *plan_win;
    const unsigned char *plan_flag;
    unsigned plan_stride;
    const unsigned *redo_static;
    AzGrav g;
};
enum { AZ_ROW_NEAR = 0, AZ_ROW_COPY = 1, AZ_ROW_ZERO = 2 };
enum { AZ_PLAN_sOc, AZ_PLAN_cOc, AZ_PLAN_sdU, AZ_PLAN_cdU, AZ_PLAN_s1U, AZ_PLAN_c1U, AZ_PLAN_NUM };
#define AZ_PLAN_OK 1u
#define AZ_PLAN_TC 2u

template <class T>
__device__ __forceinline__ void az_put3(T *o, const double r[3])
{
    o[0] = (T)r[0];
    o[1] = (T)r[1];
    o[2] = (T)r[2];
}
typedef double az_d2s __attribute__((ext_vector_type(2), aligned(8)));
typedef float az_f3s __attribute__((ext_vector_type(3), aligned(4)));
#ifndef AZ_ROWS_NT
#define AZ_ROWS_NT 1
#endif
__device__ __forceinline__ void az_put3_stream(double *o, const double r[3])
{
#if AZ_ROWS_NT
    const az_d2s a = {r[0], r[1]};
    __builtin_nontemporal_store(a, reinterpret_cast<az_d2s *>(o));
    __builtin_nontemporal_store(r[2], o + 2);
#else
    az_put3(o, r);
#endif
}
__device__ __forceinline__ void az_put3_stream(float *o, const double r[3])
{
#if AZ_ROWS_NT
    const az_f3s a = {(float)r[0], (float)r[1], (float)r[2]};
    __builtin_nontemporal_store(a, reinterpret_cast<az_f3s *>(o));
#else
    az_put3(o, r);
#endif
}

__device__ __forceinline__ void az_epilogue(double r[3], double v[3], int mode, bool vel, const double *sin_g,
                                            const double *cos_g, unsigned i)
{
    if (mode != 0) {
        const double sg = sin_g[i], cg = cos_g[i];
        az_to_ecef(r, sg, cg);
        if (vel) az_to_ecef(v, sg, cg);
        if (mode == 2) az_ecef_to_geodetic(r);
    }
}
template <bool VEL>
__device__ __forceinline__ void az_epilogue_topo(double r[3], double v[3], const PropArgs &p, unsigned i)
{
    const double sg = p.sin_g[i], cg = p.cos_g[i];
    az_to_ecef(r, sg, cg);
    if (VEL) az_to_ecef(v, sg, cg);
    az_topocentric<VEL>(r, v, *p.obs);
}

#define AZ_TM_ROW 256
#define AZ_SM_ROW (AZ_SM_CHUNK * 3 + 1)

typedef double az_d2 __attribute__((ext_vector_type(2)));

#if defined(AZ_STORE_POLICY) && AZ_STORE_POLICY == 1
#define AZ_ST1(ptr, val) __builtin_nontemporal_store((val), (ptr))
#define AZ_ST2(ptr, val) __builtin_nontemporal_store((val), (ptr))
#else
#define AZ_ST1(ptr, val) (*(ptr) = (val))
#define AZ_ST2(ptr, val) (*(ptr) = (val))
#endif

__device__ __forceinline__ double az_readlane_f64(double x, unsigned lane_uniform)
{
    const int lo = __builtin_amdgcn_readlane(__double2loint(x), (int)lane_uniform);
    const int hi = __builtin_amdgcn_readlane(__double2hiint(x), (int)lane_uniform);
    return __hiloint2double(hi, lo);
}

__device__ __forceinline__ void az_wave_lds_fence()
{
    __builtin_amdgcn_fence(__ATOMIC_RELEASE, "wavefront");
    __builtin_amdgcn_wave_barrier();
    __builtin_amdgcn_fence(__ATOMIC_ACQUIRE, "wavefront");
}

__device__ __forceinline__ void az_tm_flush(const double *L, double *row, size_t pitch, unsigned lane, unsigned par, bool last)
{
    const az_d2 *lp = reinterpret_cast<const az_d2 *>(L);
    az_d2 *g = reinterpret_cast<az_d2 *>(row);
// ... 319 lines not shown
    const unsigned sub = ITEMS ? (blockIdx.x % AZ_ONE_LISTS) : 0u;
    const unsigned n_work = ITEMS ? items[32u * sub] * (AZ_ONE_SEG / 64u) : 1u;
#pragma unroll 1
    for (unsigned w = ITEMS ? blockIdx.x / AZ_ONE_LISTS : 0u; w < n_work; w += ITEMS ? gridDim.x / AZ_ONE_LISTS : 1u) {
    const unsigned i = ITEMS ? items[AZ_ONE_HEAD + sub * list_cap + w / (AZ_ONE_SEG / 64u)] * AZ_ONE_SEG + (w % (AZ_ONE_SEG / 64u)) * 64u + threadIdx.x
                             : blockIdx.x * 64 + threadIdx.x;
    if (ITEMS && i - threadIdx.x >= n) continue;
    const double t = tsince[i < n ? i : n - 1] + (offsets ? offsets[sat] : 0.0);
    const unsigned fl = flags[sat];
    double r[3], v[3];
    int rc = AZ_FLAG_ERR(fl);
    if (rc == 0) {
        if (fl & AZ_FLAG_DEEP) {
            Sdp4Lane e;
            Sdp4Carry c;
            __shared__ double cold_deep[D_NUM * 64];
            double *cold = cold_deep + threadIdx.x;
            az_load_sdp4(el, n_pad, sat, fl, e, ColdLds{cold});
            c.atime = 0.0;
            c.xli = e(H_xlamo);
            c.xni = e(H_no_unkozai);
            rc = az_sdp4_step<true>(e, ColdLds{cold}, g, az_rotk(), t, c, r, v);
        } else {
            Sgp4Lane e;
            Sgp4Carry c;
            ColdRegs cold;
            az_load_sgp4(el, n_pad, sat, fl, e, cold);
            c.t_prev = 0.0;
            az_sgp4_step<true>(e, cold, el, n_pad, sat, g, az_rotk(), t, true, c, r, v);
        }
    }
    if (rc != 0) {
        r[0] = r[1] = r[2] = nan_on_error ? __builtin_nan("") : 0.0;
        v[0] = v[1] = v[2] = 0.0;
    }
    if (i < n) {
        if (interleaved) {
            double *o = pos + (size_t)i * 6;
            o[0] = r[0]; o[1] = r[1]; o[2] = r[2]; o[3] = v[0]; o[4] = v[1]; o[5] = v[2];
        } else {
            pos[(size_t)i * 3] = r[0]; pos[(size_t)i * 3 + 1] = r[1]; pos[(size_t)i * 3 + 2] = r[2];
            if (vel) { vel[(size_t)i * 3] = v[0]; vel[(size_t)i * 3 + 1] = v[1]; vel[(size_t)i * 3 + 2] = v[2]; }
        }
        if (err) err[i] = (unsigned char)rc;
    }
    }
}

struct PlanArgs {
    const double *el;
    const unsigned *flags;
    size_t n_pad;
    const unsigned *list;
    unsigned n_list, n_circ, n_times, tile_c, tile_e, by_flags;
    unsigned f32_mixed;
    const double *times, *offsets, *inc;
    double step, dt_mult, delta_max, grid_t0;
    double *win;
    unsigned char *flag;
    unsigned *redo_static, *redo_c0, *redo_c1, *redo_items;
    AzGrav g;
};
__global__ void __launch_bounds__(256) k_plan_windows(PlanArgs a)
{
    const unsigned slot = blockIdx.x * 256 + threadIdx.x;
    const unsigned seg = blockIdx.y;
    if (slot >= a.n_list) return;
    const unsigned s = a.list[slot];
    const unsigned fl = a.flags[s];
    const bool ecc = a.by_flags ? AZ_FLAG_ECLASS(fl) != 0 : slot >= a.n_circ;
    const unsigned tile = ecc ? a.tile_e : a.tile_c;
    const unsigned t_lo = seg * tile;
    if (t_lo >= a.n_times) return;
    const unsigned t_hi = min(t_lo + tile, a.n_times);
    const double t_first = a.grid_t0 + (a.offsets ? a.offsets[s] : 0.0);
    const double w_a = fma((double)t_lo, a.step, t_first), w_b = fma((double)(t_hi - 1), a.step, t_first);
    FastK k0, k1;
    az_load_fast(a.el, a.n_pad, s, fl, a.inc, 0, k0);
    const double dt_mult = ecc ? 64.0 : a.dt_mult;
    if (dt_mult == 128.0) az_double_increments(k0);
    az_fast_window(a.el, a.n_pad, s, w_a, w_b, dt_mult * a.step, k0);
    az_load_fast(a.el, a.n_pad, s, fl, a.inc, 1, k1);
    az_fast_window(a.el, a.n_pad, s, w_a, w_b, a.step, k1);
    bool ok = ecc ? az_fast_window_ok<true>(k0, a.g, w_a, w_b, a.delta_max) : az_fast_window_ok<false>(k0, a.g, w_a, w_b, a.delta_max);
    if (!ecc && AZ_FLAG_ECLASS(fl) != 0) ok = false;
    if (!ecc && a.f32_mixed && !az_fast32p_window_ok(k0, w_a, w_b)) ok = false;
    const size_t at = (size_t)seg * a.n_list + slot;
    double *w = a.win + at * AZ_PLAN_NUM;
    w[AZ_PLAN_sOc] = k0.sOc_; w[AZ_PLAN_cOc] = k0.cOc_; w[AZ_PLAN_sdU] = k0.sdU_; w[AZ_PLAN_cdU] = k0.cdU_;
    w[AZ_PLAN_s1U] = k1.sdU_; w[AZ_PLAN_c1U] = k1.cdU_;
    a.flag[at] = (unsigned char)((ok ? AZ_PLAN_OK : 0u) | (k0.tc_ != 0.0 ? AZ_PLAN_TC : 0u));
    if (!ok) {
        const unsigned k = atomicAdd(a.redo_static, 1u);
        a.redo_items[3 * (size_t)k + 0] = slot;
        a.redo_items[3 * (size_t)k + 1] = t_lo;
        a.redo_items[3 * (size_t)k + 2] = t_hi;
    }
}
__global__ void k_plan_arm(unsigned *redo_static, unsigned *c0, unsigned *c1)
{
    if (threadIdx.x == 0 && blockIdx.x == 0) *c0 = *c1 = *redo_static;
}
template <class K>
__device__ __forceinline__ bool az_plan_window(const PropArgs &p, unsigned seg, unsigned slot, double w_a, double w_b, K &k0)
{
    const size_t at = (size_t)seg * p.plan_stride + slot;
    const double *w = p.plan_win + at * AZ_PLAN_NUM;
    const unsigned f = p.plan_flag[at];
    k0.tmid_ = 0.5 * (w_a + w_b);
    k0.tc_ = (f & AZ_PLAN_TC) ? k0.tmid_ : 0.0;
    k0.sOc_ = w[AZ_PLAN_sOc]; k0.cOc_ = w[AZ_PLAN_cOc]; k0.sdU_ = w[AZ_PLAN_sdU]; k0.cdU_ = w[AZ_PLAN_cdU];
    return (f & AZ_PLAN_OK) != 0;
}

AZ_DEVICE double az_uniform(double x)
{
#ifdef AZ_HOST_EMUL
    return x;
#else
    return __hiloint2double(__builtin_amdgcn_readfirstlane(__double2hiint(x)),
                            __builtin_amdgcn_readfirstlane(__double2loint(x)));
#endif
}
AZ_DEVICE float az_uniform32(float x)
{
#ifdef AZ_HOST_EMUL
    return x;
#else
    return __int_as_float(__builtin_amdgcn_readfirstlane(__float_as_int(x)));
#endif
}
__device__ __forceinline__ const double *az_opaque_lds(const double *p)
{
    typedef __attribute__((address_space(3))) const double lds_cdouble;
    lds_cdouble *q = (lds_cdouble *)p;
    asm volatile("" : "+v"(q));
    return (const double *)q;
}
struct ColdBroadcast;
struct ColdBroadcast {
    double *p;
    const double *m = nullptr;
    __device__ __forceinline__ double operator()(int k) const { return p[k]; }
    __device__ __forceinline__ void set(int k, double v) const { p[k] = v; }
    __device__ __forceinline__ double mc(int k) const { return m[k]; }
    __device__ __forceinline__ ColdBroadcast fresh() const;
};
struct ColdBroadcastLit {
    double *p;
    __device__ __forceinline__ double operator()(int k) const { return p[k]; }
    __device__ __forceinline__ void set(int k, double v) const { p[k] = v; }
    __device__ __forceinline__ double mc(int k) const { return az_mc_literal(k); }
    __device__ __forceinline__ const ColdBroadcastLit &fresh() const { return *this; }
};
__device__ const double az_mc_table[MC_NUM] = AZ_MC_VALUES;
__device__ const double az_rc_table[RC_NUM] = AZ_RC_VALUES;
#define AZ_SC_NUM (MC_C5 + 1)
#define AZ_FAST_TABLE ((FCX_NUM + RC_NUM + AZ_SC_NUM + 1) & ~1)
struct McLds {
    const double *p;
    __device__ __forceinline__ double mc(int k) const { return p[k]; }
};
__device__ __forceinline__ void az_fill_fast_table(double *table, const double *__restrict__ rec, unsigned lane)
{
    static_assert(FCX_NUM + RC_NUM + AZ_SC_NUM <= 64, "one lane per table entry");
    const double *src = lane < FCX_NUM ? rec + lane
                        : lane < FCX_NUM + RC_NUM ? az_rc_table + (lane - FCX_NUM) : az_mc_table + (lane - (FCX_NUM + RC_NUM));
    if (lane < FCX_NUM + RC_NUM + AZ_SC_NUM) table[lane] = *src;
}
__device__ __forceinline__ ColdBroadcast ColdBroadcast::fresh() const { return ColdBroadcast{p, az_opaque_lds(m)}; }
#ifndef AZ_ROWSF_WAVES
#define AZ_ROWSF_WAVES 6
#endif
#ifndef AZ_ROWSF32_WAVES
#define AZ_ROWSF32_WAVES 4
#endif
#ifndef AZ_ROWSF32P_WAVES
#define AZ_ROWSF32P_WAVES 3
#endif
#ifndef AZ_ROWSF_ECC_WAVES
#define AZ_ROWSF_ECC_WAVES 4
#endif
#ifndef AZ_ROWS_TLDS
#define AZ_ROWS_TLDS 1024
#endif

enum { AZ_SINK_F64 = 0, AZ_SINK_F32 = 1, AZ_SINK_SCREEN = 2 };

__device__ __forceinline__ void az_wave_argmin(double &d2, unsigned &t)
{
#pragma unroll
    for (int off = 32; off > 0; off >>= 1) {
        const double od = __shfl_xor(d2, off, 64);
        const unsigned ot = __shfl_xor(t, off, 64);
        if (od < d2 || (od == d2 && ot < t)) {
            d2 = od;
            t = ot;
        }
    }
}


#ifndef AZ_ROWS_LDS_STORE
#define AZ_ROWS_LDS_STORE 1
#endif
typedef float az_f4 __attribute__((ext_vector_type(4)));
template <class T>
__device__ __forceinline__ void az_stage3(T *stage, unsigned lane, const double r[3])
{
    stage[lane * 3 + 0] = (T)r[0];
    stage[lane * 3 + 1] = (T)r[1];
    stage[lane * 3 + 2] = (T)r[2];
}
typedef unsigned az_u4 __attribute__((ext_vector_type(4)));
struct AzRowSink {
    __amdgpu_buffer_rsrc_t pos, vel;
};
template <class T>
__device__ __forceinline__ AzRowSink az_row_sink(T *prow, T *vrow, unsigned n_times)
{
    const unsigned row_bytes = n_times * 3u * (unsigned)sizeof(T);
    return AzRowSink{__builtin_amdgcn_make_buffer_rsrc(prow, 0, row_bytes, 0x00020000),
                     __builtin_amdgcn_make_buffer_rsrc(vrow ? vrow : prow, 0, row_bytes, 0x00020000)};
}
#ifndef AZ_AUX_NT
#define AZ_AUX_NT 2
#endif
template <bool VEL, class T>
__device__ __forceinline__ void az_flush_stage(const T *stage, const AzRowSink &sink, unsigned base, unsigned lane)
{
    constexpr unsigned PIECES = 64 * 3 * sizeof(T) / 16;
    constexpr int aux = AZ_ROWS_NT ? AZ_AUX_NT : 0;
    const az_u4 *src = reinterpret_cast<const az_u4 *>(stage) + lane;
    const unsigned voff = lane * 16u, soff = base * 3u * (unsigned)sizeof(T);
    if constexpr (PIECES >= 64) {
        const az_u4 a = src[0];
        __builtin_amdgcn_raw_buffer_store_b128(a, sink.pos, voff, soff, aux);
        if (VEL) {
            const az_u4 c = src[PIECES];
            __builtin_amdgcn_raw_buffer_store_b128(c, sink.vel, voff, soff, aux);
        }
        if (lane < PIECES - 64) {
            const az_u4 b = src[64];
            __builtin_amdgcn_raw_buffer_store_b128(b, sink.pos, voff + 1024u, soff, aux);
            if (VEL) {
                const az_u4 d = src[PIECES + 64];
                __builtin_amdgcn_raw_buffer_store_b128(d, sink.vel, voff + 1024u, soff, aux);
            }
        }
    } else if (lane < PIECES) {
        const az_u4 a = src[0];
        __builtin_amdgcn_raw_buffer_store_b128(a, sink.pos, voff, soff, aux);
        if (VEL) {
            const az_u4 c = src[PIECES];
            __builtin_amdgcn_raw_buffer_store_b128(c, sink.vel, voff, soff, aux);
        }
// ... 28 lines not shown
                                                    const double *tsince, unsigned n, double *pos, double *vel, unsigned char *err,
                                                    AzGrav g, const double *offsets, unsigned *items, unsigned list_cap)
{
    const unsigned lane = threadIdx.x, seg = blockIdx.x, lo = seg * AZ_ONE_SEG;
    const unsigned cnt = min((unsigned)AZ_ONE_SEG, n - lo);
    const unsigned fl = flags[sat];
    __shared__ float dl_lds[AZ_ONE_SEG];
    __shared__ __attribute__((aligned(16))) double rows_stage[2 * 64 * 3];
    const double off = az_uniform(offsets ? offsets[sat] : 0.0);
    const bool ecc = AZ_FLAG_ECLASS(fl) != 0;
    bool ok = AZ_FLAG_ERR(fl) == 0 && !(fl & AZ_FLAG_DEEP) && cnt >= 128u;
    double t0 = 0.0, step = 0.0;
    FastK k;
    if (ok) {
        t0 = az_uniform(tsince[lo]) + off;
        step = ((az_uniform(tsince[lo + cnt - 1]) + off) - t0) / (double)(cnt - 1u);
        bool far = false;
#pragma unroll 4
        for (unsigned j = lane; j < (unsigned)AZ_ONE_SEG; j += 64u) {
            const unsigned jj = min(j, cnt - 1u);
            const double d = (tsince[lo + jj] + off) - fma((double)jj, step, t0);
            dl_lds[j] = (float)d;
            far |= !(fabs(d) <= AZ_DELTA_MAX);
        }
        ok = !az_any(far) && step != 0.0 && fabs(step) * (double)cnt <= 3000.0;
    }
    if (ok) {
#define L(f) el[(size_t)F_##f * n_pad + sat]
        double sdA, cdA, sdW, cdW;
        az_sincos(L(mdot) * (64.0 * step), sdA, cdA);
        az_sincos(L(argpdot) * (64.0 * step), sdW, cdW);
#undef L
        az_load_fast_with(el, n_pad, sat, fl, sdA, cdA, sdW, cdW, k);
        const double w_a = t0, w_b = fma((double)(cnt - 1u), step, t0);
        az_fast_window(el, n_pad, sat, w_a, w_b, 64.0 * step, k);
        ok = ecc ? az_fast_window_ok<true>(k, g, w_a, w_b, AZ_DELTA_MAX) : az_fast_window_ok<false>(k, g, w_a, w_b, AZ_DELTA_MAX);
    }
    if (ok) {
        FastCarry fc;
        az_seed_fast(el, n_pad, sat, fma((double)lane - 64.0, step, t0), k.tc_, fc);
        double *prow = pos + (size_t)lo * 3, *vrow = VEL ? vel + (size_t)lo * 3 : nullptr;
        const bool staged = ((reinterpret_cast<size_t>(prow) | (VEL ? reinterpret_cast<size_t>(vrow) : 0)) & 15u) == 0;
        const AzRowSink sink = az_row_sink(prow, vrow, cnt);
        az_wave_lds_fence();
#pragma unroll 1
        for (unsigned base = 0; base < cnt; base += 64u) {
            const unsigned i = base + lane;
            const bool live = i < cnt;
            const double dl = (double)dl_lds[i];
            const double t = fma((double)i, step, t0) + dl;
            double r[3], v[3];
            const bool bad = ecc ? az_sgp4_fast_step<VEL, true, 1>(k, g, RotCoefLit(), t, fc, r, v, dl)
                                 : az_sgp4_fast_step<VEL, false, 1>(k, g, RotCoefLit(), t, fc, r, v, dl);
            if (az_any(bad && live)) {
                ok = false;
                break;
            }
            az_rows_store<VEL>(staged, base + 64u <= cnt, live, lane, rows_stage, prow, vrow, base, r, v, sink);
            if (err && live) err[lo + i] = 0;
        }
    }
    if (!ok && lane == 0) {
        const unsigned sub = seg % AZ_ONE_LISTS;
        items[AZ_ONE_HEAD + sub * list_cap + atomicAdd(items + 32u * sub, 1u)] = seg;
    }
}

#define AZ_FRAME_SEG 256
template <bool VEL, int FRAME, int SINK, bool ECC, int DELTA = 0>
__global__ void __launch_bounds__(64, FRAME >= 2 ? 4 : (ECC ? AZ_ROWSF_ECC_WAVES : (FRAME == 1 || DELTA == 2 ? 5 : AZ_ROWSF_WAVES))) k_rows_fast(PropArgs p)
{
    typedef typename std::conditional<SINK == AZ_SINK_F32, float, double>::type out_t;
    const unsigned lane = threadIdx.x;
    const unsigned row = az_list_slot(p);
    [[maybe_unused]] const AzObserver obs = FRAME == 3 ? *p.obs : AzObserver{};
    if (row >= az_list_end(p)) return;
    const unsigned s = p.list[row];
    if (SINK != AZ_SINK_SCREEN && ((p.mask != nullptr && p.mask[s] == 0) || s < p.row_lo || s >= p.row_hi)) return;
    const unsigned t_lo = blockIdx.y * p.tile;
    if (t_lo >= p.n_times) return;
    const unsigned t_hi = min(t_lo + p.tile, p.n_times);
    unsigned base = t_lo;
    bool window_ok;
    double best_d2 = __builtin_inf();
    unsigned best_t = 0xffffffffu;
    {
        __shared__ __attribute__((aligned(16))) double cold_lds[AZ_FAST_TABLE];
        __shared__ __attribute__((aligned(16))) out_t rows_stage[AZ_ROWS_LDS_STORE ? 2 * 64 * 3 : 4];
        const double off = az_uniform(p.offsets ? p.offsets[s] : 0.0);
        const double *__restrict__ rec = p.fast_rec + (size_t)s * FR_NUM;
        az_fill_fast_table(cold_lds, rec, lane);
        const size_t out_row = p.rows_compact ? (size_t)p.ecc_row0 + row : (size_t)s;
        out_t *prow = SINK == AZ_SINK_SCREEN ? nullptr : reinterpret_cast<out_t *>(p.pos) + out_row * p.n_times * 3;
        out_t *vrow = VEL ? reinterpret_cast<out_t *>(p.vel) + out_row * p.n_times * 3 : nullptr;
        const bool staged = AZ_ROWS_LDS_STORE && SINK != AZ_SINK_SCREEN &&
                            (((reinterpret_cast<size_t>(prow) | (VEL ? reinterpret_cast<size_t>(vrow) : 0)) & 15u) == 0);
        FastKBcast k;
        {
            const double w_a = fma((double)t_lo, p.uniform_step, p.grid_t0 + off), w_b = fma((double)(t_hi - 1), p.uniform_step, p.grid_t0 + off);
            window_ok = az_plan_window(p, blockIdx.y, row + p.redo_slot0, w_a, w_b, k);
            if (!window_ok) return;
            az_fast_rec_hot(rec, k);
            az_wave_lds_fence();
            if (DELTA && k.tc_ != 0.0 && lane == 0) cold_lds[FCX_udot] = fma(2.0 * rec[FC_nl2], k.tc_, rec[FCX_udot]);
        }
        typedef typename std::conditional<DELTA == 2, double, float>::type dl_t;
        __shared__ dl_t dl_lds[DELTA ? AZ_DELTA_SEG : 1];
        if (DELTA) {
            const dl_t *src = DELTA == 2 ? reinterpret_cast<const dl_t *>(p.delta64) : reinterpret_cast<const dl_t *>(p.delta);
#pragma unroll
            for (unsigned j = lane; j < AZ_DELTA_SEG; j += 64) dl_lds[j] = src[t_lo + j];
        }
        az_wave_lds_fence();
        const double step = p.uniform_step;
        const double t_first = p.grid_t0 + off;
        FastCarry fc;
        az_seed_fast_rec(rec, rec[FC_nl2], fma((double)(t_lo + lane) - 64.0, step, t_first), k.tc_, fc,
                         McLds{cold_lds + FCX_NUM + RC_NUM});
        __shared__ double gst_lds[FRAME ? 2 * AZ_FRAME_SEG : 2];
        if (FRAME) {
#pragma unroll
            for (unsigned j = lane; j < AZ_FRAME_SEG; j += 64) {
                const unsigned jj = min(t_lo + j, p.n_times - 1);
                gst_lds[2 * j] = p.sin_g[jj];
                gst_lds[2 * j + 1] = p.cos_g[jj];
            }
            az_wave_lds_fence();
        }
        AzRowSink sink{};
        if constexpr (SINK != AZ_SINK_SCREEN) sink = az_row_sink(prow, vrow, p.n_times);
#pragma unroll 1
        for (; window_ok && base < t_hi; base += 64) {
            const unsigned i = base + lane;
            const bool live = i < t_hi;
            double t = fma((double)i, step, t_first), dl = 0.0;
            if (DELTA) {
                dl = (double)dl_lds[i - t_lo];
                t += dl;
            }
            const double *cold_now = az_opaque_lds(cold_lds);
            k.cold = cold_now;
            const RotCoefLds rk{cold_now + FCX_NUM};
            double r[3], v[3];
#if defined(AZ_ABLATE) && AZ_ABLATE == 2
            r[0] = t; r[1] = t + 1.0; r[2] = t + 2.0; v[0] = t + 3.0; v[1] = t + 4.0; v[2] = t + 5.0;
#else
            const bool bad = az_sgp4_fast_step<VEL, ECC, DELTA>(k, p.g, rk, t, fc, r, v, dl);
            if (az_any(bad && live)) break;
#endif
            if (SINK == AZ_SINK_SCREEN) {
                const double *q = p.screen_target + (size_t)(live ? i : t_hi - 1) * 3;
                const double dx = q[0] - r[0], dy = q[1] - r[1], dz = q[2] - r[2];
                const double d2 = fma(dx, dx, fma(dy, dy, dz * dz));
                if (live && d2 < best_d2) {
                    best_d2 = d2;
                    best_t = i;
                }
                continue;
            }
            if (FRAME) {
                if (((base - t_lo) & (AZ_FRAME_SEG - 1u)) == 0u && base != t_lo) {
                    az_wave_lds_fence();
#pragma unroll
                    for (unsigned j = lane; j < AZ_FRAME_SEG; j += 64) {
                        const unsigned jn = min(base + j, p.n_times - 1);
                        gst_lds[2 * j] = p.sin_g[jn];
                        gst_lds[2 * j + 1] = p.cos_g[jn];
                    }
                    az_wave_lds_fence();
                }
                const unsigned jj = (i - t_lo) & (AZ_FRAME_SEG - 1u);
                const double sg = gst_lds[2 * jj], cg = gst_lds[2 * jj + 1];
                az_to_ecef(r, sg, cg);
                if (VEL) az_to_ecef(v, sg, cg);
                if (FRAME == 2) az_ecef_to_geodetic(r);
                if (FRAME == 3) az_topocentric<VEL>(r, v, obs);
            }
#if defined(AZ_ABLATE) && AZ_ABLATE == 1
            if (!(live && (r[0] + r[1] + r[2] + (VEL ? v[0] + v[1] + v[2] : 0.0)) == 1.2345e300)) continue;
#endif
            az_rows_store<VEL>(staged, base + 64 <= t_hi, live, lane, rows_stage, prow, vrow, base, r, v, sink);
        }
    }
    if (SINK == AZ_SINK_SCREEN) {
        az_wave_argmin(best_d2, best_t);
        if (lane == 0) {
            p.part_d2[(size_t)blockIdx.y * p.plan_stride + row + p.redo_slot0] = best_d2;
            p.part_t[(size_t)blockIdx.y * p.plan_stride + row + p.redo_slot0] = best_t;
        }
    }
    if (ECC && base < t_hi && lane == 0) {
        const unsigned k = atomicAdd(p.redo_count, 1u);
        p.redo_items[3 * (size_t)k + 0] = row + p.redo_slot0;
        p.redo_items[3 * (size_t)k + 1] = base;
        p.redo_items[3 * (size_t)k + 2] = t_hi;
    }
}

#define AZ_TILE_SATS 16
#define AZ_TILE_SEG_MAX 1024
#define AZ_TILE_PITCH 49
template <bool VEL, int FRAME = 0, int DELTA = 0>
__global__ void __launch_bounds__(1024, 1) k_tiles_fast(PropArgs p)
{
    constexpr unsigned NA = VEL ? 2u : 1u;
    constexpr bool ECEF = FRAME != 0;
    [[maybe_unused]] const AzObserver obs = FRAME == 3 ? *p.obs : AzObserver{};
    __shared__ __attribute__((aligned(16))) double cold_all[AZ_TILE_SATS * AZ_FAST_TABLE];
    __shared__ __attribute__((aligned(16))) double tile[2 * NA * 64 * AZ_TILE_PITCH];
    __shared__ double gst[ECEF ? 2 * AZ_TILE_SEG_MAX : 2];
    const unsigned lane = threadIdx.x & 63u, w = __builtin_amdgcn_readfirstlane(threadIdx.x >> 6);
    double *cold_lds = cold_all + w * AZ_FAST_TABLE;
    const unsigned tile_id = az_xcd_row();
    const unsigned s_first = tile_id * AZ_TILE_SATS;
    if (s_first >= p.n_rows) return;
    const unsigned n_valid = min((unsigned)AZ_TILE_SATS, p.n_rows - s_first);
    const bool have = w < n_valid;
    const unsigned s = s_first + (have ? w : 0u);
    const unsigned fl = p.flags[s];
    const unsigned rm = p.rowmap[s], kind = rm >> 30, slot = rm & 0x3fffffffu;
    const unsigned t_lo = blockIdx.y * p.tile, t_hi = min(t_lo + p.tile, p.n_times);
    const bool in_window = have && s >= p.row_lo && s < p.row_hi && (p.mask == nullptr || p.mask[s] != 0);
    __shared__ unsigned writable_lds;
    if (threadIdx.x == 0) writable_lds = 0u;
    __syncthreads();
    if (lane == 0 && in_window) atomicOr(&writable_lds, 1u << w);
    __syncthreads();
    const unsigned writable = writable_lds;
    if (writable == 0u) return;
    const bool contig = writable == 0xffffu;
    bool dead = !(in_window && kind == AZ_ROW_NEAR);
    const bool copy = in_window && kind == AZ_ROW_COPY, zero = in_window && kind == AZ_ROW_ZERO;
    if (ECEF) {
        for (unsigned j = threadIdx.x; j < t_hi - t_lo; j += 1024u) {
            gst[2 * j] = p.sin_g[t_lo + j];
            gst[2 * j + 1] = p.cos_g[t_lo + j];
        }
    }
    const bool ecc = AZ_FLAG_ECLASS(fl) != 0;
    const double off = az_uniform(p.offsets ? p.offsets[s] : 0.0);
    const double step = p.uniform_step, t_first = p.grid_t0 + off;
    typedef double dl_t;
    __shared__ dl_t dl_lds[DELTA ? AZ_DELTA_SEG : 1];
    if (DELTA) {
        const dl_t *src = p.delta64;
        if (threadIdx.x < AZ_DELTA_SEG) dl_lds[threadIdx.x] = src[t_lo + threadIdx.x];
        if (!ECEF) __syncthreads();
    }
    if (ECEF) __syncthreads();
    FastKBcast k;
    FastCarry fc;
    if (!dead) {
        const double *__restrict__ rec = p.fast_rec + (size_t)s * FR_NUM;
        az_fill_fast_table(cold_lds, rec, lane);
        const double w_a = fma((double)t_lo, step, t_first), w_b = fma((double)(t_hi - 1), step, t_first);
        if (!az_plan_window(p, blockIdx.y, slot, w_a, w_b, k)) dead = true;
        az_fast_rec_hot(rec, k);
        az_wave_lds_fence();
        if (DELTA && k.tc_ != 0.0 && lane == 0) cold_lds[FCX_udot] = fma(2.0 * rec[FC_nl2], k.tc_, rec[FCX_udot]);
        az_wave_lds_fence();
        az_seed_fast_rec(rec, rec[FC_nl2], fma((double)(t_lo + lane) - 64.0, step, t_first), k.tc_, fc, McLds{cold_lds + FCX_NUM + RC_NUM});
    }
    unsigned f_lds[3], f_out[3], f_row = 0;
#pragma unroll
    for (unsigned m = 0; m < 3; ++m) {
// ... 842 lines not shown
```

bindings/zig/astroz_hip.zig:

```

pub const HipError = error{
    BadTleLength,
    BadChecksum,
    DeepSpaceNotSupported,
    InvalidEccentricity,
    SatelliteDecayed,
    ValueError,
    OutOfMemory,
    NullPointer,
    NotInitialized,
    DeviceFailure,
    Unknown,
};

pub fn check(rc: i32) HipError!void {
    return switch (rc) {
        0 => {},
        -1 => HipError.BadTleLength,
        -2 => HipError.BadChecksum,
        -10 => HipError.DeepSpaceNotSupported,
        -11 => HipError.InvalidEccentricity,
        -12 => HipError.SatelliteDecayed,
        -20 => HipError.ValueError,
        -100 => HipError.OutOfMemory,
// ... 7 lines not shown
pub const Handle = opaque {};

pub const Err = enum(i32) {
    ok = 0,
    bad_tle_length = -1,
    bad_checksum = -2,
    deep_space_not_supported = -10,
    invalid_eccentricity = -11,
    satellite_decayed = -12,
    value_error = -20,
    alloc_failed = -100,
    null_pointer = -101,
    not_initialized = -102,
    hip = -200,
    unknown = -999,
};

pub extern "c" fn azh_device_count() c_int;
pub extern "c" fn azh_last_error() [*:0]const u8;
pub extern "c" fn azh_parse_tle_lines(line1: [*:0]const u8, line2: [*:0]const u8, out16: [*]f64) i32;
pub extern "c" fn azh_constellation_from_tle_text(text: [*]const u8, len: usize, grav: i32, device: i32, out: *?*Handle) i32;
pub extern "c" fn azh_constellation_from_tle_lines(line1: [*]const [*:0]const u8, line2: [*]const [*:0]const u8, n: usize, grav: i32, device: i32, out: *?*Handle) i32;
pub extern "c" fn azh_constellation_from_elements(n: usize, epoch_jd: [*]const f64, mm_revday: [*]const f64, ecc: [*]const f64, incl_deg: [*]const f64, raan_deg: [*]const f64, argp_deg: [*]const f64, ma_deg: [*]const f64, bstar: [*]const f64, grav: i32, device: i32, out: *?*Handle) i32;
pub extern "c" fn azh_constellation_free(h: ?*Handle) void;
pub extern "c" fn azh_num_satellites(h: ?*const Handle) usize;
pub extern "c" fn azh_num_sgp4(h: ?*const Handle) usize;
pub extern "c" fn azh_num_sdp4(h: ?*const Handle) usize;
pub extern "c" fn azh_get_epochs(h: ?*const Handle, out: [*]f64) i32;
pub extern "c" fn azh_get_status(h: ?*const Handle, err: ?[*]u8, is_deep: ?[*]u8, irez: ?[*]u8) i32;
pub extern "c" fn azh_get_field(h: ?*const Handle, name: [*:0]const u8, out: [*]f64) i32;
pub extern "c" fn azh_propagate_host(h: ?*Handle, times_min: [*]const f64, n_times: usize, epoch_offsets_min: ?[*]const f64, pos: [*]f64, vel: ?[*]f64, output_mode: i32, reference_jd: f64, sat_mask: ?[*]const u8, layout: i32, out_stride_sats: usize, err: ?[*]u8) i32;
pub extern "c" fn azh_propagate_device(h: ?*Handle, times_min: [*]const f64, n_times: usize, epoch_offsets_min: ?[*]const f64, d_pos: [*]f64, d_vel: ?[*]f64, output_mode: i32, reference_jd: f64, sat_mask: ?[*]const u8, layout: i32, out_stride_sats: usize, d_err: ?[*]u8, stream: ?*anyopaque) i32;
pub extern "c" fn azh_propagate_device_cached(h: ?*Handle, d_pos: [*]f64, d_vel: ?[*]f64, layout: i32, out_stride_sats: usize, d_err: ?[*]u8, stream: ?*anyopaque) i32;
pub extern "c" fn azh_propagate_jd_host(h: ?*Handle, jd: [*]const f64, fr: [*]const f64, n_times: usize, pos: [*]f64, vel: ?[*]f64, output_mode: i32, layout: i32, err: ?[*]u8) i32;
pub extern "c" fn azh_propagate_one_host(h: ?*Handle, sat_index: usize, tsince_min: [*]const f64, n: usize, pos: [*]f64, vel: ?[*]f64, err: ?[*]u8) i32;
pub extern "c" fn azh_synchronize(h: ?*Handle) i32;
pub extern "c" fn azh_set_time_tile(h: ?*Handle, sgp4_tile: u32, sdp4_tile: u32) i32;
pub extern "c" fn azh_set_timing(h: ?*Handle, enabled: i32) i32;
pub extern "c" fn azh_last_kernel_ms(h: ?*Handle) f64;

pub extern "c" fn azh_propagate_device_f32(h: ?*Handle, times_min: [*]const f64, n_times: usize, epoch_offsets_min: ?[*]const f64,
    d_pos: [*]f32, d_vel: ?[*]f32, output_mode: i32, reference_jd: f64, sat_mask: ?[*]const u8, layout: i32,
    out_stride_sats: usize, d_err: ?[*]u8, stream: ?*anyopaque) i32;
pub extern "c" fn azh_propagate_device_cached_f32(h: ?*Handle, d_pos: [*]f32, d_vel: ?[*]f32, layout: i32,
    out_stride_sats: usize, d_err: ?[*]u8, stream: ?*anyopaque) i32;

pub extern "c" fn azh_screen_target_host(h: ?*Handle, times_min: [*]const f64, n_times: usize, epoch_offsets_min: ?[*]const f64,
    target_index: usize, threshold_km: f64, reference_jd: f64, min_dist_km: [*]f64, min_t_index: [*]u32) i32;
pub extern "c" fn azh_screen_target_device(h: ?*Handle, times_min: [*]const f64, n_times: usize, epoch_offsets_min: ?[*]const f64,
    target_index: usize, threshold_km: f64, reference_jd: f64, d_min_dist_km: [*]f64, d_min_t_index: [*]u32, stream: ?*anyopaque) i32;
pub extern "c" fn azh_screen_track_device(h: ?*Handle, times_min: [*]const f64, n_times: usize, epoch_offsets_min: ?[*]const f64,
    d_track: [*]const f64, exclude_index: usize, threshold_km: f64, d_min_dist_km: [*]f64, d_min_t_index: [*]u32, stream: ?*anyopaque) i32;
pub extern "c" fn azh_coarse_screen_device(d_pos: [*]const f64, n_sats: usize, n_times: usize, layout: i32, stride_sats: usize,
    threshold_km: f64, valid_mask: ?[*]const u8, out_pairs: [*]u32, out_t_index: [*]u32, max_results: usize, n_found: *usize,
    stream: ?*anyopaque) i32;
pub extern "c" fn azh_coarse_screen_host(pos: [*]const f64, n_sats: usize, n_times: usize, layout: i32, stride_sats: usize,
    threshold_km: f64, valid_mask: ?[*]const u8, out_pairs: [*]u32, out_t_index: [*]u32, max_results: usize, n_found: *usize,
    device: i32) i32;
pub extern "c" fn azh_screen_all_host(h: ?*Handle, times_min: [*]const f64, n_times: usize, epoch_offsets_min: ?[*]const f64,
    threshold_km: f64, out_pairs: [*]u32, out_t_index: [*]u32, max_results: usize, n_found: *usize) i32;

pub extern "c" fn azh_parse_tle_text(text: [*]const u8, len: usize, out16: [*]f64, max_records: usize, n_found: *usize) i32;
pub extern "c" fn azh_parse_omm_json(text: [*]const u8, len: usize, out16: [*]f64, max_records: usize, n_found: *usize) i32;
pub extern "c" fn azh_set_parse_threads(n: i32) void;
pub extern "c" fn azh_constellation_from_omm_json(text: [*]const u8, len: usize, grav: i32, device: i32, out: *?*Handle) i32;
pub extern "c" fn azh_constellation_subset(h: ?*const Handle, indices: [*]const u32, n: usize, device: i32, out: *?*Handle) i32;

pub extern "c" fn azh_propagate_device_window(h: ?*Handle, row_lo: usize, row_hi: usize, d_pos: [*]f64, d_vel: ?[*]f64, layout: i32,
    out_stride_sats: usize, d_err: ?[*]u8, stream: ?*anyopaque) i32;
pub extern "c" fn azh_set_f32_mode(h: ?*Handle, mode: i32) i32;
pub extern "c" fn azh_set_f32_arithmetic(h: ?*Handle, enabled: i32) i32;
pub extern "c" fn azh_set_fast_path(h: ?*Handle, enabled: i32) i32;
pub extern "c" fn azh_set_tile_kernel(h: ?*Handle, enabled: i32) i32;
pub extern "c" fn azh_set_graphs(h: ?*Handle, enabled: i32) i32;
pub extern "c" fn azh_set_host_points(n: usize) void;
pub extern "c" fn azh_get_host_points() usize;
pub extern "c" fn azh_set_host_copy_threads(n: i32) void;
pub extern "c" fn azh_host_alloc(bytes: usize, out: *?*anyopaque) i32;
pub extern "c" fn azh_host_free(p: ?*anyopaque) void;
pub extern "c" fn azh_host_pool_stats(live_bytes: ?*usize, free_bytes: ?*usize) void;
pub extern "c" fn azh_host_pool_trim() void;
pub extern "c" fn azh_last_path(h: ?*const Handle) u32;
pub extern "c" fn azh_last_one_stats(h: ?*Handle, n_segments: ?*u32, n_handed_over: ?*u32) i32;
pub extern "c" fn azh_propagate_one_device(h: ?*Handle, sat_index: usize, d_tsince_min: [*]const f64, n: usize, d_pos: [*]f64,
    d_vel: ?[*]f64, d_err: ?[*]u8, stream: ?*anyopaque) i32;
pub extern "c" fn azh_selftest_math(x: [*]const f64, n: usize, out6n: [*]f64, device: i32) i32;
pub extern "c" fn azh_selftest_host_step(el: [*]const f64, n_pad: usize, sat: usize, flags: u32, grav: i32, tsince_min: [*]const f64, n: usize,
    out6n: [*]f64, err: ?[*]u8) i32;
pub extern "c" fn azh_selftest_coords(op: i32, in: *const [4]f64, out: *[5]f64) i32;

pub extern "c" fn coords_julian_to_gmst(jd: f64) f64;
pub extern "c" fn coords_eci_to_ecef(eci: *const [3]f64, gmst: f64, ecef: *[3]f64) void;
pub extern "c" fn coords_ecef_to_geodetic(ecef: *const [3]f64, lla: *[3]f64) void;
pub extern "c" fn azh_coords_topocentric(r_teme: *const [3]f64, v_teme: ?*const [3]f64, gmst: f64, observer_lla: *const [3]f64,
    aer: *[3]f64, aer_rate: ?*[3]f64) void;

pub const OUT_TOPOCENTRIC: i32 = 3;
pub const Pass = extern struct {
    t_rise_min: f64,
    t_culm_min: f64,
    t_set_min: f64,
    max_elevation_rad: f64,
    rise_azimuth_rad: f64,
    set_azimuth_rad: f64,
    flags: u32,
    grid_rise: u32,
    grid_culm: u32,
    grid_set: u32,
};
pub const PASS_UP_AT_START: u32 = 1;
pub const PASS_UP_AT_END: u32 = 2;
pub const PASS_CUT_BY_ERROR: u32 = 4;
pub extern "c" fn azh_set_observer(h: ?*Handle, lat_deg: f64, lon_deg: f64, alt_km: f64) i32;
pub extern "c" fn azh_find_passes_host(h: ?*Handle, times_min: [*]const f64, n_times: usize, epoch_offsets_min: ?[*]const f64,
    reference_jd: f64, min_elevation_deg: f64, out: [*]Pass, max_passes: usize, n_passes: [*]u32) i32;
pub extern "c" fn azh_find_passes_device(h: ?*Handle, times_min: [*]const f64, n_times: usize, epoch_offsets_min: ?[*]const f64,
    reference_jd: f64, min_elevation_deg: f64, d_out: [*]Pass, max_passes: usize, d_n_passes: [*]u32, stream: ?*anyopaque) i32;
pub extern "c" fn azh_find_passes_stations_host(h: ?*Handle, times_min: [*]const f64, n_times: usize,
    epoch_offsets_min: ?[*]const f64, reference_jd: f64, stations_lla: [*]const [3]f64, min_elevation_deg: [*]const f64,
    n_stations: usize, out: [*]Pass, max_passes: usize, n_passes: [*]u32) i32;
pub extern "c" fn azh_find_passes_stations_device(h: ?*Handle, times_min: [*]const f64, n_times: usize,
    epoch_offsets_min: ?[*]const f64, reference_jd: f64, stations_lla: [*]const [3]f64, min_elevation_deg: [*]const f64,
    n_stations: usize, d_out: [*]Pass, max_passes: usize, d_n_passes: [*]u32, stream: ?*anyopaque) i32;

pub const Coverage = extern struct {
    mean_in_view: f64,
    max_gap_min: f64,
    n_covered: u32,
    min_in_view: u32,
    max_in_view: u32,
    n_gaps: u32,
    grid_gap_start: u32,
    grid_gap_end: u32,
    flags: u32,
    reserved: u32,
};
pub const COVERAGE_GAP_AT_START: u32 = 1;
pub const COVERAGE_GAP_AT_END: u32 = 2;
pub extern "c" fn azh_coverage_host(h: ?*Handle, times_min: [*]const f64, n_times: usize, epoch_offsets_min: ?[*]const f64,
    reference_jd: f64, points_lla: [*]const [3]f64, min_elevation_deg: [*]const f64, n_points: usize, min_satellites: u32,
    stats: [*]Coverage, counts_or_null: ?[*]u32) i32;
pub extern "c" fn azh_coverage_device(h: ?*Handle, times_min: [*]const f64, n_times: usize, epoch_offsets_min: ?[*]const f64,
    reference_jd: f64, points_lla: [*]const [3]f64, min_elevation_deg: [*]const f64, n_points: usize, min_satellites: u32,
    d_stats: [*]Coverage, d_counts_or_null: ?[*]u32, stream: ?*anyopaque) i32;

pub extern "c" fn azh_sun_position_teme(jd: f64, sun_km: *[3]f64) void;
pub extern "c" fn azh_selftest_sun(jd: [*]const f64, n: usize, out3n: [*]f64, device: i32) i32;
pub extern "c" fn azh_shadow_state(r_teme: *const [3]f64, sun_km: *const [3]f64, f_umbra: ?*f64, f_penumbra: ?*f64) i32;
pub const Eclipse = extern struct {
    t_entry_min: f64,
    t_exit_min: f64,
    flags: u32,
    grid_entry: u32,
    grid_exit: u32,
    reserved: u32,
};
pub const ECLIPSE_IN_AT_START: u32 = 1;
pub const ECLIPSE_IN_AT_END: u32 = 2;
pub const ECLIPSE_CUT_BY_ERROR: u32 = 4;
pub const SHADOW_UMBRA: i32 = 0;
pub const SHADOW_PENUMBRA: i32 = 1;
pub extern "c" fn azh_find_eclipses_host(h: ?*Handle, times_min: [*]const f64, n_times: usize, epoch_offsets_min: ?[*]const f64,
    reference_jd: f64, kind: i32, out: ?[*]Eclipse, max_eclipses: usize, n_eclipses: [*]u32, state_or_null: ?[*]u8) i32;
pub extern "c" fn azh_find_eclipses_device(h: ?*Handle, times_min: [*]const f64, n_times: usize, epoch_offsets_min: ?[*]const f64,
    reference_jd: f64, kind: i32, d_out: ?[*]Eclipse, max_eclipses: usize, d_n_eclipses: [*]u32, d_state_or_null: ?[*]u8,
    stream: ?*anyopaque) i32;
// ... 64 lines not shown
```

include/astroz_hip.h:

```cpp
#ifndef ASTROZ_HIP_H
#define ASTROZ_HIP_H

#include <stddef.h>
#include <stdint.h>

#ifdef __cplusplus
extern "C" {
#endif

enum {
    AZ_OK = 0,
    AZ_ERR_BAD_TLE_LENGTH = -1,
    AZ_ERR_BAD_CHECKSUM = -2,
    AZ_ERR_DEEP_SPACE_NOT_SUPPORTED = -10,
    AZ_ERR_INVALID_ECCENTRICITY = -11,
    AZ_ERR_SATELLITE_DECAYED = -12,
    AZ_ERR_VALUE = -20,
    AZ_ERR_ALLOC_FAILED = -100,
    AZ_ERR_NULL_POINTER = -101,
    AZ_ERR_NOT_INITIALIZED = -102,
    AZ_ERR_HIP = -200,
    AZ_ERR_UNKNOWN = -999
};

// ... 203 lines not shown
int32_t azh_screen_target_device(azh_constellation *c, const double *times_min, size_t n_times,
                                 const double *epoch_offsets_min, size_t target_index, double threshold_km,
                                 double reference_jd, double *d_min_dist_km, uint32_t *d_min_t_index, void *stream);

int32_t azh_screen_track_device(azh_constellation *c, const double *times_min, size_t n_times,
                                const double *epoch_offsets_min, const double *d_track, size_t exclude_index,
                                double threshold_km, double *d_min_dist_km, uint32_t *d_min_t_index, void *stream);

int32_t azh_coarse_screen_device(const double *d_pos, size_t n_sats, size_t n_times, int32_t layout,
                                 size_t stride_sats, double threshold_km, const uint8_t *valid_mask,
                                 uint32_t *out_pairs, uint32_t *out_t_index, size_t max_results, size_t *n_found,
                                 void *stream);
int32_t azh_coarse_screen_host(const double *pos, size_t n_sats, size_t n_times, int32_t layout, size_t stride_sats,
                               double threshold_km, const uint8_t *valid_mask, uint32_t *out_pairs,
                               uint32_t *out_t_index, size_t max_results, size_t *n_found, int32_t device);
int32_t azh_screen_all_host(azh_constellation *c, const double *times_min, size_t n_times,
                            const double *epoch_offsets_min, double threshold_km, uint32_t *out_pairs,
                            uint32_t *out_t_index, size_t max_results, size_t *n_found);

typedef struct azh_group azh_group;
int32_t azh_group_create_from_tle_text(const char *text, size_t len, int32_t grav, const int32_t *devices,
                                       int32_t n_devices, int32_t n_chunks, azh_group **out);
int32_t azh_group_create_from_omm_json(const char *text, size_t len, int32_t grav, const int32_t *devices,
                                       int32_t n_devices, int32_t n_chunks, azh_group **out);
void azh_group_free(azh_group *g);
size_t azh_group_num_satellites(const azh_group *g);
int32_t azh_group_num_devices(const azh_group *g);
size_t azh_group_padded_rows(const azh_group *g);
int32_t azh_group_get_epochs(const azh_group *g, double *out_n);
int32_t azh_group_propagate_host(azh_group *g, const double *times_min, size_t n_times, const double *epoch_offsets_min,
                                 size_t n_offsets, double *pos, double *vel, int32_t output_mode, double reference_jd,
                                 uint8_t *err);
int32_t azh_group_propagate_allgather(azh_group *g, const double *times_min, size_t n_times,
                                      const double *epoch_offsets_min, size_t n_offsets, double *const *d_pos,
                                      double *const *d_vel);

int32_t azh_group_screen_target_host(azh_group *g, const double *times_min, size_t n_times, const double *epoch_offsets_min,
                                     size_t n_offsets, size_t target_index, double threshold_km, double reference_jd,
                                     double *min_dist_km, uint32_t *min_t_index);
int32_t azh_group_screen_target_device(azh_group *g, const double *times_min, size_t n_times, const double *epoch_offsets_min,
                                       size_t n_offsets, size_t target_index, double threshold_km, double reference_jd,
                                       double *const *d_min_dist_km, uint32_t *const *d_min_t_index);
size_t azh_group_shard_size(const azh_group *g, int32_t device_slot);
int32_t azh_group_shard_rows(const azh_group *g, int32_t device_slot, uint32_t *out_rows);
int32_t azh_group_synchronize(azh_group *g);

int32_t azh_propagate_jd_host(azh_constellation *c, const double *jd, const double *fr, size_t n_times,
                              double *pos, double *vel, int32_t output_mode, int32_t layout, uint8_t *err);
int32_t azh_synchronize(azh_constellation *c);

int32_t azh_propagate_one_host(azh_constellation *c, size_t sat_index, const double *tsince_min, size_t n,
                               double *pos, double *vel, uint8_t *err);

int32_t azh_propagate_one_device(azh_constellation *c, size_t sat_index, const double *d_tsince_min, size_t n,
                                 double *d_pos, double *d_vel, uint8_t *d_err, void *stream);
int32_t azh_selftest_math(const double *x, size_t n, double *out6n, int32_t device);
int32_t azh_selftest_coords(int32_t op, const double in[4], double out[5]);
int32_t azh_selftest_host_step(const double *el, size_t n_pad, size_t sat, uint32_t flags, int32_t grav, const double *tsince_min,
                               size_t n, double *out6n, uint8_t *err);

int32_t azh_set_time_tile(azh_constellation *c, uint32_t sgp4_tile, uint32_t sdp4_tile);
int32_t azh_set_fast_path(azh_constellation *c, int32_t enabled);
int32_t azh_set_tile_kernel(azh_constellation *c, int32_t enabled);
int32_t azh_set_graphs(azh_constellation *c, int32_t enabled);
void azh_set_host_copy_threads(int32_t n);
void azh_set_host_points(size_t n);
size_t azh_get_host_points(void);
int32_t azh_host_alloc(size_t bytes, void **out);
void azh_host_free(void *p);
void azh_host_pool_stats(size_t *live_bytes, size_t *free_bytes);
void azh_host_pool_trim(void);
int32_t azh_set_timing(azh_constellation *c, int32_t enabled);
double azh_last_kernel_ms(azh_constellation *c);
#define AZH_PATH_ROWS_FAST 1u
#define AZH_PATH_TILES_FAST 2u
#define AZH_PATH_ROWS_GENERIC 4u
#define AZH_PATH_LANE_SAT 8u
#define AZH_PATH_DEEP_ROWS 16u
#define AZH_PATH_COLS_FAST 64u
#define AZH_PATH_QUASI_UNIFORM 32u
#define AZH_PATH_HOST_STEP 128u
uint32_t azh_last_path(const azh_constellation *c);
int32_t azh_last_one_stats(azh_constellation *c, uint32_t *n_segments, uint32_t *n_handed_over);

#ifdef __cplusplus
}
#endif
#endif
```

Before: 92.47 billion.

## Add per-window accuracy tiers to use a cheaper eps rotation in fast rows

The window planner now classifies each satellite-window into a tier. Windows whose Kepler-iteration correction eps is bounded small get a specialised fast step that replaces the 16th-angle rotation with a tiny-angle rotation. The row kernel dispatches on the stored tier through a templated lambda, and it adds a min-eccentricity check that lets the em clamp be dropped. The position and velocity output is also refactored to save a few multiplies, and a diagnostic API is added to count windows per tier. The trade-off is more code variants, a possible loss of occupancy, and extra window rejections from the new eccentricity floor.

```diff
diff --git a/astroz_amd/_native.py b/astroz_amd/_native.py
--- a/astroz_amd/_native.py
+++ b/astroz_amd/_native.py
@@ -42,7 +42,7 @@
     "azh_num_satellites", "azh_num_sgp4", "azh_num_sdp4", "azh_get_epochs", "azh_get_status",
     "azh_get_field", "azh_propagate_host", "azh_propagate_device", "azh_propagate_device_cached", "azh_propagate_device_window",
     "azh_propagate_jd_host", "azh_synchronize", "azh_propagate_one_host", "azh_set_time_tile", "azh_set_timing", "azh_set_fast_path", "azh_set_tile_kernel", "azh_set_graphs", "azh_set_f32_arithmetic", "azh_set_f32_mode",
-    "azh_last_kernel_ms", "azh_last_path", "azh_last_one_stats", "azh_set_host_copy_threads", "azh_set_host_points", "azh_get_host_points", "azh_selftest_coords", "azh_selftest_host_step", "azh_host_alloc", "azh_host_free", "azh_host_pool_stats", "azh_host_pool_trim", "azh_propagate_device_f32", "azh_propagate_device_cached_f32",
+    "azh_last_kernel_ms", "azh_last_path", "azh_last_one_stats", "azh_last_window_tiers", "azh_set_host_copy_threads", "azh_set_host_points", "azh_get_host_points", "azh_selftest_coords", "azh_selftest_host_step", "azh_host_alloc", "azh_host_free", "azh_host_pool_stats", "azh_host_pool_trim", "azh_propagate_device_f32", "azh_propagate_device_cached_f32",
     "azh_screen_target_host", "azh_screen_target_device", "azh_coarse_screen_device", "azh_coarse_screen_host",
     "azh_screen_all_host", "azh_constellation_from_omm_json", "azh_propagate_one_device", "azh_selftest_math",
     "azh_parse_tle_text", "azh_parse_omm_json", "azh_set_parse_threads", "coords_julian_to_gmst",
@@ -250,6 +250,8 @@
     L.azh_last_path.restype = u32
     L.azh_last_one_stats.argtypes = [vp, vp, vp]
     L.azh_last_one_stats.restype = C.c_int32
+    L.azh_last_window_tiers.argtypes = [vp, vp]
+    L.azh_last_window_tiers.restype = C.c_int32
     L.azh_propagate_device_f32.argtypes = L.azh_propagate_device.argtypes
     L.azh_propagate_device_f32.restype = i32
     L.azh_propagate_device_cached_f32.argtypes = L.azh_propagate_device_cached.argtypes
@@ -692,6 +694,12 @@
         return int(a.value), int(b.value)
 
 
+    def last_window_tiers(self):
+        cnt = (C.c_uint32 * 4)()
+        check(lib().azh_last_window_tiers(self._h, cnt), "azh_last_window_tiers")
+        return dict(zip(("general", "eps", "ecc", "rejected"), (int(x) for x in cnt)))
+
+
 class DeviceGroup:
 
     def __init__(self, text, devices, grav=WGS72, n_chunks=4):
diff --git a/astroz_amd/csrc/astroz_hip.hip b/astroz_amd/csrc/astroz_hip.hip
--- a/astroz_amd/csrc/astroz_hip.hip
+++ b/astroz_amd/csrc/astroz_hip.hip
@@ -197,6 +197,7 @@
         DevBuf<unsigned char> flag;
         DevBuf<unsigned> redo;
     } plan[4];
+    int last_plan = -1;
     DevBuf<double> d_inc;
     DevBuf<double> d_fast_rec;
     double uniform_step = 0.0;
@@ -267,6 +268,7 @@
         unsigned fails;
         hipGraph_t graph;
         hipGraphExec_t exec;
+        int plan = -1;
     };
     std::vector<LaunchGraph> graphs;
     int graphs_on = 0;
@@ -773,6 +775,7 @@
     c->seeds_valid = false;
     drop_graphs(c);
     for (auto &pl : c->plan) pl.valid = false;
+    c->last_plan = -1;
     c->uniform_step = 0.0;
     c->delta_max = 0.0;
     c->delta_wide = false;
@@ -894,6 +897,7 @@
             pl.flag.ensure((size_t)n_list * n_seg) != AZ_OK)
             return AZ_ERR_HIP;
         HIP_TRY(hipMemsetAsync(pl.redo.p, 0, 4 * sizeof(unsigned), st));
+        HIP_TRY(hipMemsetAsync(pl.flag.p, 0, (size_t)n_list * n_seg, st));
         PlanArgs q{};
         q.el = a.el; q.flags = a.flags; q.n_pad = a.n_pad; q.list = a.list; q.n_list = n_list; q.n_circ = a.n_circ;
         q.n_times = a.n_times; q.tile_c = shape.tile_c; q.tile_e = shape.tile_e; q.by_flags = shape.kind == 2 ? 1u : 0u;
@@ -910,6 +914,7 @@
         pl.valid = true;
         pl.tile_c = shape.tile_c; pl.tile_e = shape.tile_e; pl.n_list = n_list; pl.n_seg = n_seg; pl.parity = 0; pl.mixed32 = shape.mixed32;
     }
+    c->last_plan = (int)shape.kind;
     a.plan_win = pl.win.p;
     a.plan_flag = pl.flag.p;
     a.plan_stride = n_list;
@@ -956,6 +961,7 @@
     if (row_lo >= row_hi) return AZ_OK;
     if (stride == 0) stride = c->n;
     if (layout == AZ_LAYOUT_TIME_MAJOR && stride < c->n) return AZ_ERR_VALUE;
+    c->last_plan = -1;
 
     PropArgs a{};
     a.el = c->d_el.p;
@@ -1130,6 +1136,7 @@
         HIP_TRY(hipGraphLaunch(hit->exec, st));
         for (unsigned k = 0; k < 4; ++k) c->plan[k].parity = (hit->sig_after >> k) & 1u;
         c->last_path = hit->path;
+        c->last_plan = hit->plan;
         HIP_TRY(hipEventRecord(c->ev_graph, st));
         return AZ_OK;
     }
@@ -1168,6 +1175,7 @@
     pending->exec = exec;
     pending->sig_after = plan_sig(c);
     pending->path = c->last_path;
+    pending->plan = c->last_plan;
     HIP_TRY(hipGraphLaunch(exec, st));
     HIP_TRY(hipEventRecord(c->ev_graph, st));
     return AZ_OK;
@@ -3079,6 +3087,31 @@
     unsigned cnt = 0;
     for (unsigned k = 0; k < AZ_ONE_LISTS; ++k) cnt += head[32u * k];
     *n_handed_over = cnt;
+    return AZ_OK;
+}
+
+int32_t azh_last_window_tiers(azh_constellation *c, uint32_t counts[AZH_WINDOW_TIER_COUNTS])
+{
+    if (!c || !counts) return AZ_ERR_NULL_POINTER;
+    for (unsigned k = 0; k < AZH_WINDOW_TIER_COUNTS; ++k) counts[k] = 0;
+    if (c->last_plan < 0 || !c->plan[c->last_plan].valid) return AZ_OK;
+    const azh_constellation::FastPlan &pl = c->plan[c->last_plan];
+    if (set_device(c) != AZ_OK) return AZ_ERR_HIP;
+    HIP_TRY(hipDeviceSynchronize());
+    std::vector<unsigned char> f;
+    try {
+        f.resize((size_t)pl.n_list * pl.n_seg);
+    } catch (const std::bad_alloc &) {
+        return AZ_ERR_HIP;
+    }
+    if (f.empty()) return AZ_OK;
+    HIP_TRY(hipMemcpy(f.data(), pl.flag.p, f.size(), hipMemcpyDeviceToHost));
+    for (unsigned char v : f) {
+        if (!(v & AZ_PLAN_SET)) continue;
+        if (!(v & AZ_PLAN_OK)) ++counts[AZH_WINDOW_TIER_REJECTED];
+        else if (v & AZ_PLAN_ECC) ++counts[AZH_WINDOW_TIER_ECC];
+        else ++counts[((v >> AZ_PLAN_TIER_SHIFT) & AZ_PLAN_TIER_MASK) ? AZH_WINDOW_TIER_EPS : AZH_WINDOW_TIER_GENERAL];
+    }
     return AZ_OK;
 }
 
diff --git a/astroz_amd/csrc/fast_step.h b/astroz_amd/csrc/fast_step.h
--- a/astroz_amd/csrc/fast_step.h
+++ b/astroz_amd/csrc/fast_step.h
@@ -323,15 +323,21 @@
 #define AZ_FAST_EL2 1.6e-5
 #define AZ_FAST_TEMP2 6.0e-4
 
+enum { AZ_TIER_GENERAL = 0, AZ_TIER_EPS = 1, AZ_TIER_NUM = 2 };
+#define AZ_TIER_EPS_MAX 0.0009765625
+#define AZ_FAST_EM_MIN 1.0e-6
+
 template <bool ECC>
-AZ_DEVICE bool az_fast_window_ok(const FastK &k, const AzGrav &g, double t_a, double t_b, double dmax = 0.0)
+AZ_DEVICE int az_fast_window_tier(const FastK &k, const AzGrav &g, double t_a, double t_b, double dmax = 0.0)
 {
     const double T = fmax(fabs(t_a), fabs(t_b)) + dmax;
     const double ae = fabs(k.eta_);
     const double th = fma(fabs(k.xmcof_), ae * fma(2.0 * ae, ae, 6.0), fabs(k.omgcof_) * T);
     const double da = T * fma(T, fma(T, fma(T, fabs(k.d4_), fabs(k.d3_)), fabs(k.d2_)), fabs(k.cc1_));
-    const double em = fabs(k.ecb_) + fma(fabs(k.bc4_), T, fabs(k.bc5_));
+    const double dem = fma(fabs(k.bc4_), T, fabs(k.bc5_));
+    const double em = fabs(k.ecb_) + dem;
     bool ok = (th <= AZ_ROT_16TH) & (da <= 0.25) & (em <= 0.9);
+    ok &= k.ecb_ - dem >= AZ_FAST_EM_MIN;
     const double sam = k.sab_ * (1.0 - da);
     const double inv_am = 1.0 / (sam * sam);
     const double temp = inv_am / fma(-em, em, 1.0);
@@ -348,10 +354,20 @@
     ok &= temp2 <= AZ_FAST_TEMP2;
     const double a_nd = fma(fabs(k.k_node_), temp2, fma(fabs(k.nodedot_), 0.5 * fabs(t_b - t_a) + dmax, fabs(k.xnodcf_) * T * T));
     ok &= a_nd <= AZ_ROT_MED;
-    return ok;
-}
-
-template <bool VEL, bool ECC = false, int DELTA = 0, class K = FastK, class RC = RotCoefLit>
+    if (!ok) return -1;
+    return (!ECC && eps <= AZ_TIER_EPS_MAX) ? AZ_TIER_EPS : AZ_TIER_GENERAL;
+}
+template <bool ECC>
+AZ_DEVICE bool az_fast_window_ok(const FastK &k, const AzGrav &g, double t_a, double t_b, double dmax = 0.0)
+{
+    return az_fast_window_tier<ECC>(k, g, t_a, t_b, dmax) >= 0;
+}
+
+#ifndef AZ_FAST_PROBE
+#define AZ_FAST_PROBE(name, value)
+#endif
+
+template <bool VEL, bool ECC = false, int DELTA = 0, int TIER = AZ_TIER_GENERAL, class K = FastK, class RC = RotCoefLit>
 AZ_DEVICE bool az_sgp4_fast_step(const K &k, const AzGrav &g, const RC &rk, double t, FastCarry &st, double r[3],
                                   double v[3], double dl = 0.0)
 {
@@ -388,7 +404,9 @@
     const double smm = fma(cA, p, fma(sA, q, sA));
     const double sw = fma(-cW, p, fma(sW, q, sW));
     const double cw = fma(sW, p, fma(cW, q, cW));
-    const double em = fmax(fma(-k.bc5(), smm, fma(-k.bc4(), t, k.ecb())), 1.0e-6);
+    const double em = fma(-k.bc5(), smm, fma(-k.bc4(), t, k.ecb()));
+    AZ_FAST_PROBE(th, th)
+    AZ_FAST_PROBE(em, em)
 
     const double sqrt_am = k.sab() * fabs(tempa);
     const double am = sqrt_am * sqrt_am;
@@ -402,8 +420,12 @@
     double s = st.sU, c = st.cU;
     {
         const double eps = fma(temp * k.xlcof(), axnl, nl);
-        az_pq_16th(eps, rk, p, q);
-        az_rot_apply2(s, c, p, q);
+        AZ_FAST_PROBE(eps, eps)
+        if constexpr (!ECC && TIER >= AZ_TIER_EPS) az_rotate_tiny2(s, c, eps, rk);
+        else {
+            az_pq_16th(eps, rk, p, q);
+            az_rot_apply2(s, c, p, q);
+        }
     }
 
     const double el2 = fma(axnl, axnl, aynl * aynl);
@@ -476,6 +498,7 @@
     const double mrt = fma(rl, fma(k.k_mrt() * temp2, betal, 1.0), k.k_c2u() * temp1 * cos2u);
     const double t2s = temp2 * sin2u;
     const double a_nd = fma(k.k_node(), t2s, fma(k.nodedot(), t - k.tmid(), k.xnodcf() * t2));
+    AZ_FAST_PROBE(a_nd, a_nd)
     double ssu = sinu, csu = cosu, sn = k.sOc(), cn = k.cOc(), si = k.sinio(), ci = k.cosio();
     az_rotate_tiny2(ssu, csu, k.k_su() * t2s, rk);
     az_pq_16th(a_nd, rk, p, q);
@@ -483,25 +506,21 @@
     az_rotate_tiny2(si, ci, k.k_inc() * temp2 * cos2u, rk);
 
     const double xmx = -sn * ci, xmy = cn * ci;
-    const double ux = fma(xmx, ssu, cn * csu);
-    const double uy = fma(xmy, ssu, sn * csu);
-    const double uz = si * ssu;
     const double rs = mrt * g.radius_km;
-    r[0] = rs * ux;
-    r[1] = rs * uy;
-    r[2] = rs * uz;
+    const double ra_s = rs * ssu, ra_c = rs * csu;
+    r[0] = fma(xmx, ra_s, cn * ra_c);
+    r[1] = fma(xmy, ra_s, sn * ra_c);
+    r[2] = si * ra_s;
     if (VEL) {
         const double rv = ra * g.vkmpersec;
         const double vk = rv * inv_ome;
         const double nxt = rv * inv_am * temp1;
         const double mvt = fma(-nxt * k.x1mth2(), sin2u, vk * esine);
         const double rvdot = fma(nxt, fma(k.x1mth2(), cos2u, k.k_rv()), vk * betal);
-        const double vx = fma(xmx, csu, -(cn * ssu));
-        const double vy = fma(xmy, csu, -(sn * ssu));
-        const double vz = si * csu;
-        v[0] = fma(mvt, ux, rvdot * vx);
-        v[1] = fma(mvt, uy, rvdot * vy);
-        v[2] = fma(mvt, uz, rvdot * vz);
+        const double va_s = fma(mvt, ssu, rvdot * csu), va_c = fma(mvt, csu, -(rvdot * ssu));
+        v[0] = fma(xmx, va_s, cn * va_c);
+        v[1] = fma(xmy, va_s, sn * va_c);
+        v[2] = si * va_s;
     }
     return bad;
 }
diff --git a/astroz_amd/csrc/kernels.h b/astroz_amd/csrc/kernels.h
--- a/astroz_amd/csrc/kernels.h
+++ b/astroz_amd/csrc/kernels.h
@@ -88,6 +88,10 @@
 enum { AZ_PLAN_sOc, AZ_PLAN_cOc, AZ_PLAN_sdU, AZ_PLAN_cdU, AZ_PLAN_s1U, AZ_PLAN_c1U, AZ_PLAN_NUM };
 #define AZ_PLAN_OK 1u
 #define AZ_PLAN_TC 2u
+#define AZ_PLAN_TIER_SHIFT 2
+#define AZ_PLAN_TIER_MASK 1u
+#define AZ_PLAN_ECC 16u
+#define AZ_PLAN_SET 32u
 
 template <class T>
 __device__ __forceinline__ void az_put3(T *o, const double r[3])
@@ -573,14 +577,16 @@
     az_fast_window(a.el, a.n_pad, s, w_a, w_b, dt_mult * a.step, k0);
     az_load_fast(a.el, a.n_pad, s, fl, a.inc, 1, k1);
     az_fast_window(a.el, a.n_pad, s, w_a, w_b, a.step, k1);
-    bool ok = ecc ? az_fast_window_ok<true>(k0, a.g, w_a, w_b, a.delta_max) : az_fast_window_ok<false>(k0, a.g, w_a, w_b, a.delta_max);
+    const int tier = ecc ? az_fast_window_tier<true>(k0, a.g, w_a, w_b, a.delta_max) : az_fast_window_tier<false>(k0, a.g, w_a, w_b, a.delta_max);
+    bool ok = tier >= 0;
     if (!ecc && AZ_FLAG_ECLASS(fl) != 0) ok = false;
     if (!ecc && a.f32_mixed && !az_fast32p_window_ok(k0, w_a, w_b)) ok = false;
     const size_t at = (size_t)seg * a.n_list + slot;
     double *w = a.win + at * AZ_PLAN_NUM;
     w[AZ_PLAN_sOc] = k0.sOc_; w[AZ_PLAN_cOc] = k0.cOc_; w[AZ_PLAN_sdU] = k0.sdU_; w[AZ_PLAN_cdU] = k0.cdU_;
     w[AZ_PLAN_s1U] = k1.sdU_; w[AZ_PLAN_c1U] = k1.cdU_;
-    a.flag[at] = (unsigned char)((ok ? AZ_PLAN_OK : 0u) | (k0.tc_ != 0.0 ? AZ_PLAN_TC : 0u));
+    a.flag[at] = (unsigned char)((ok ? AZ_PLAN_OK | ((unsigned)tier << AZ_PLAN_TIER_SHIFT) : 0u) | (k0.tc_ != 0.0 ? AZ_PLAN_TC : 0u) |
+                                 (ecc ? AZ_PLAN_ECC : 0u) | AZ_PLAN_SET);
     if (!ok) {
         const unsigned k = atomicAdd(a.redo_static, 1u);
         a.redo_items[3 * (size_t)k + 0] = slot;
@@ -593,7 +599,7 @@
     if (threadIdx.x == 0 && blockIdx.x == 0) *c0 = *c1 = *redo_static;
 }
 template <class K>
-__device__ __forceinline__ bool az_plan_window(const PropArgs &p, unsigned seg, unsigned slot, double w_a, double w_b, K &k0)
+__device__ __forceinline__ bool az_plan_window(const PropArgs &p, unsigned seg, unsigned slot, double w_a, double w_b, K &k0, unsigned *tier = nullptr)
 {
     const size_t at = (size_t)seg * p.plan_stride + slot;
     const double *w = p.plan_win + at * AZ_PLAN_NUM;
@@ -601,6 +607,7 @@
     k0.tmid_ = 0.5 * (w_a + w_b);
     k0.tc_ = (f & AZ_PLAN_TC) ? k0.tmid_ : 0.0;
     k0.sOc_ = w[AZ_PLAN_sOc]; k0.cOc_ = w[AZ_PLAN_cOc]; k0.sdU_ = w[AZ_PLAN_sdU]; k0.cdU_ = w[AZ_PLAN_cdU];
+    if (tier) *tier = (f >> AZ_PLAN_TIER_SHIFT) & AZ_PLAN_TIER_MASK;
     return (f & AZ_PLAN_OK) != 0;
 }
 
@@ -663,6 +670,9 @@
 #ifndef AZ_ROWSF_WAVES
 #define AZ_ROWSF_WAVES 6
 #endif
+#ifndef AZ_ROWS_TIERS
+#define AZ_ROWS_TIERS 1
+#endif
 #ifndef AZ_ROWSF32_WAVES
 #define AZ_ROWSF32_WAVES 4
 #endif
@@ -857,6 +867,7 @@
     const unsigned t_hi = min(t_lo + p.tile, p.n_times);
     unsigned base = t_lo;
     bool window_ok;
+    unsigned tier = AZ_TIER_GENERAL;
     double best_d2 = __builtin_inf();
     unsigned best_t = 0xffffffffu;
     {
@@ -873,7 +884,7 @@
         FastKBcast k;
         {
             const double w_a = fma((double)t_lo, p.uniform_step, p.grid_t0 + off), w_b = fma((double)(t_hi - 1), p.uniform_step, p.grid_t0 + off);
-            window_ok = az_plan_window(p, blockIdx.y, row + p.redo_slot0, w_a, w_b, k);
+            window_ok = az_plan_window(p, blockIdx.y, row + p.redo_slot0, w_a, w_b, k, &tier);
             if (!window_ok) return;
             az_fast_rec_hot(rec, k);
             az_wave_lds_fence();
@@ -904,8 +915,10 @@
         }
         AzRowSink sink{};
         if constexpr (SINK != AZ_SINK_SCREEN) sink = az_row_sink(prow, vrow, p.n_times);
+        auto run = [&](auto tier_c, const unsigned t_end) __attribute__((always_inline)) {
+        constexpr int TIER = decltype(tier_c)::value;
 #pragma unroll 1
-        for (; window_ok && base < t_hi; base += 64) {
+        for (; window_ok && base < t_end; base += 64) {
             const unsigned i = base + lane;
             const bool live = i < t_hi;
             double t = fma((double)i, step, t_first), dl = 0.0;
@@ -920,7 +933,7 @@
 #if defined(AZ_ABLATE) && AZ_ABLATE == 2
             r[0] = t; r[1] = t + 1.0; r[2] = t + 2.0; v[0] = t + 3.0; v[1] = t + 4.0; v[2] = t + 5.0;
 #else
-            const bool bad = az_sgp4_fast_step<VEL, ECC, DELTA>(k, p.g, rk, t, fc, r, v, dl);
+            const bool bad = az_sgp4_fast_step<VEL, ECC, DELTA, TIER>(k, p.g, rk, t, fc, r, v, dl);
             if (az_any(bad && live)) break;
 #endif
             if (SINK == AZ_SINK_SCREEN) {
@@ -956,6 +969,9 @@
 #endif
             az_rows_store<VEL>(staged, base + 64 <= t_hi, live, lane, rows_stage, prow, vrow, base, r, v, sink);
         }
+        };
+        if constexpr (AZ_ROWS_TIERS && !ECC && FRAME == 0) run(std::integral_constant<int, AZ_TIER_EPS>(), tier == AZ_TIER_EPS ? t_hi : t_lo);
+        run(std::integral_constant<int, AZ_TIER_GENERAL>(), t_hi);
     }
     if (SINK == AZ_SINK_SCREEN) {
         az_wave_argmin(best_d2, best_t);
diff --git a/bindings/zig/astroz_hip.zig b/bindings/zig/astroz_hip.zig
--- a/bindings/zig/astroz_hip.zig
+++ b/bindings/zig/astroz_hip.zig
@@ -113,6 +113,7 @@
 pub extern "c" fn azh_host_pool_trim() void;
 pub extern "c" fn azh_last_path(h: ?*const Handle) u32;
 pub extern "c" fn azh_last_one_stats(h: ?*Handle, n_segments: ?*u32, n_handed_over: ?*u32) i32;
+pub extern "c" fn azh_last_window_tiers(h: ?*Handle, counts: *[4]u32) i32;
 pub extern "c" fn azh_propagate_one_device(h: ?*Handle, sat_index: usize, d_tsince_min: [*]const f64, n: usize, d_pos: [*]f64,
     d_vel: ?[*]f64, d_err: ?[*]u8, stream: ?*anyopaque) i32;
 pub extern "c" fn azh_selftest_math(x: [*]const f64, n: usize, out6n: [*]f64, device: i32) i32;
diff --git a/include/astroz_hip.h b/include/astroz_hip.h
--- a/include/astroz_hip.h
+++ b/include/astroz_hip.h
@@ -309,6 +309,12 @@
 #define AZH_PATH_HOST_STEP 128u
 uint32_t azh_last_path(const azh_constellation *c);
 int32_t azh_last_one_stats(azh_constellation *c, uint32_t *n_segments, uint32_t *n_handed_over);
+#define AZH_WINDOW_TIER_GENERAL 0
+#define AZH_WINDOW_TIER_EPS 1
+#define AZH_WINDOW_TIER_ECC 2
+#define AZH_WINDOW_TIER_REJECTED 3
+#define AZH_WINDOW_TIER_COUNTS 4
+int32_t azh_last_window_tiers(azh_constellation *c, uint32_t counts[AZH_WINDOW_TIER_COUNTS]);
 
 #ifdef __cplusplus
 }
```

Result: faster. 94.51 billion, median of 6 (+2.2%).
